# QData/ChromeGCN

Measured on AMD Instinct MI355X. Metric: GCN windows/sec (2-layer, d_model=128) on GM12878 Hi-C graph, higher is better.
Workload: dtype f32

## Files before the change

chromegcn_amd/_lib.py:

```python
import ctypes
import os

import torch

from . import _build

_c_int = ctypes.c_int
_c_vp = ctypes.c_void_p
_c_sz = ctypes.c_size_t
_c_float = ctypes.c_float
_c_uint = ctypes.c_uint

_TYPES = {"i": _c_int, "u": _c_uint, "ll": ctypes.c_longlong, "z": _c_sz, "f": _c_float, "zp": ctypes.POINTER(_c_sz)}
_HEADER = {
    "cgcn_abi_version": (_c_int, ""),
    "cgcn_strerror": (ctypes.c_char_p, "code:i"),
    "cgcn_spmm": (_c_int, "stream n_rows:i n_cols:i S:i d:i rowptr col val row_scale X Y aux"),
    "cgcn_layer_fwd": (_c_int, "stream n:i S:i d:i rowptr col val row_scale X W b wg cg Xn Z H gate dropout_p:f rng_state "
                               "stream_id:u H_in colstats colstats_rows:i aux"),
    "cgcn_layer_fwd_colstats_plan": (_c_int, "n:i S:i d:i mode:i rows_per_tile"),
    "cgcn_debug_set_fwd_split_bytes": (None, "bytes:ll"),
    "cgcn_debug_set_products": (None, "mode:i"),
    "cgcn_debug_get_products": (_c_int, ""),
    "cgcn_debug_layer_fwd_route": (_c_int, "n:i S:i d:i aux colstats_rows:i"),
    "cgcn_debug_layer_bwd_route": (_c_int, "n:i S:i d:i"),
    "cgcn_layer_bwd_workspace_bytes": (_c_sz, "n:i S:i d:i"),
    "cgcn_layer_bwd": (_c_int, "stream n:i S:i d:i rowptr_t col_t val_t row_scale X Z H gate W wg dXn dgate dX dHs dW db dwg "
                               "dcg accumulate:i in_dropout_p:f rng_state in_stream_id:u head workspace workspace_bytes:z "
                               "aux_stream sgd aux_t"),
    "cgcn_debug_layer_bwd_phases": (_c_int, "stream n:i S:i d:i rowptr_t col_t val_t row_scale X Z H gate W wg dXn dgate dX dHs "
                                            "dW db dwg dcg accumulate:i in_dropout_p:f rng_state in_stream_id:u head workspace "
                                            "workspace_bytes:z phases:i aux_t"),
    "cgcn_head_workspace_bytes": (_c_sz, "n:i S:i d:i C:i"),
    "cgcn_head_workspace_layout": (_c_int, "n:i S:i d:i C:i dym_offset:zp bnc_offset:zp part_offset:zp"),
    "cgcn_head_bwd_partials": (_c_int, "n:i"),
    "cgcn_head_fwd": (_c_int, "stream n:i S:i d:i C:i X bn_w bn_b run_mean run_var num_batches_tracked momentum:f eps:f "
                              "training:i W_out b_out target dropout_p:f rng_state probs loss dpred save_mean save_invstd "
                              "workspace workspace_bytes:z"),
    "cgcn_head_logits": (_c_int, "stream n:i S:i d:i C:i X bn_w bn_b run_mean run_var eps:f W_out b_out logits"),
    "cgcn_head_train": (_c_int, "stream n:i S:i d:i C:i X bn_w bn_b run_mean run_var num_batches_tracked momentum:f eps:f "
                                "W_out b_out target dropout_p:f rng_state probs loss save_mean save_invstd col_stats "
                                "col_stats_tiles:i col_stats_rows:i workspace workspace_bytes:z"),
    "cgcn_debug_head_train_phases": (_c_int, "stream n:i S:i d:i C:i X bn_w bn_b run_mean run_var num_batches_tracked "
                                             "momentum:f eps:f W_out b_out target dropout_p:f rng_state probs loss save_mean "
                                             "save_invstd col_stats col_stats_tiles:i col_stats_rows:i workspace "
                                             "workspace_bytes:z phases:i"),
    "cgcn_head_bwd": (_c_int, "stream n:i S:i d:i C:i X bn_w bn_b save_mean save_invstd W_out dpred dloss dropout_p:f "
                              "rng_state dX dW_out db_out dbn_w dbn_b accumulate:i workspace workspace_bytes:z"),
    "cgcn_sddmm": (_c_int, "stream n:i S:i d:i rowptr col A B out accumulate:i"),
    "cgcn_saliency_normalize": (_c_int, "stream n:i rowptr val raw out"),
    "cgcn_graph_count": (_c_int, "stream n:i adj_type:i rowptr_in col_in val_in row_counts rowptr_out"),
    "cgcn_graph_fill": (_c_int, "stream n:i adj_type:i rowptr_in col_in val_in rowptr_out col_out val_out row_scale "
                                "symmetric_flag"),
    "cgcn_metrics_workspace_bytes": (_c_sz, "n:ll C:i"),
    "cgcn_multilabel_metrics": (_c_int, "stream n:ll C:i probs targets fdr_cutoff:f out workspace workspace_bytes:z"),
    "cgcn_multilabel_metrics_nonneg": (_c_int, "stream n:ll C:i probs targets fdr_cutoff:f out bad workspace "
                                               "workspace_bytes:z"),
    "cgcn_sgd_step": (_c_int, "stream count:ll param grad momentum_buf lr:f momentum:f weight_decay:f nesterov:i "
                              "grad_scale:f rng_state"),
    "cgcn_adam_step": (_c_int, "stream count:ll param grad exp_avg exp_avg_sq step n_step:i ticket lr:f beta1:f beta2:f "
                               "eps:f weight_decay:f grad_scale:f rng_state"),
    "cgcn_ablation_prepare": (_c_int, "stream n:i C:i targets label_bits pos_lists pos_ranks pos_counts"),
    "cgcn_ablation_workspace_bytes": (_c_sz, "n_inst:i S:i d:i layers:i"),
    "cgcn_ablation_layer": (_c_int, "stream n:i S:i d:i rowptr col val row_scale X X_inst W b wg cg label_bits C:i pos_list "
                                    "pos_rank n_pos:i cols n_cols:i X_out removed"),
    "cgcn_ablation_head": (_c_int, "stream n:i S:i d:i C:i X X_inst bn_w bn_b run_mean run_var eps:f W_out b_out pos_lists "
                                   "pos_counts label:i n_pos:i cols n_cols:i removed base M"),
    "cgcn_ablation_mask": (_c_int, "stream n:i C:i rowptr col val row_scale label_bits label_i:i label_j:i val_out "
                                   "row_scale_out removed"),
    "cgcn_ablation_reduce": (_c_int, "stream n:i S:i C:i logits pos_lists pos_counts label:i col_label:i removed base M"),
    "cgcn_hic_workspace_bytes": (_c_sz, "M:ll N:i capacity:ll K:ll"),
    "cgcn_hic_count": (_c_int, "stream M:ll pos1 pos2 window_start N:i workspace workspace_bytes:z n_survivors"),
    "cgcn_hic_build": (_c_int, "stream M:ll pos1 pos2 count norm n_bins:ll resolution_bp:i window_start N:i K:ll capacity:ll "
                               "workspace workspace_bytes:z rowptr_out col_out nnz_out n_survivors"),
    "cgcn_hic_up_workspace_bytes": (_c_sz, "M:ll N:i capacity:ll K:ll resolution_bp:i window_bp:i n_window_bins:ll"),
    "cgcn_hic_count_up": (_c_int, "stream M:ll pos1 pos2 window_start N:i resolution_bp:i window_bp:i n_window_bins:ll workspace "
                                  "workspace_bytes:z n_survivors"),
    "cgcn_hic_build_up": (_c_int, "stream M:ll pos1 pos2 count norm n_bins:ll resolution_bp:i window_bp:i n_window_bins:ll "
                                  "window_start N:i K:ll capacity:ll workspace workspace_bytes:z rowptr_out col_out nnz_out "
                                  "n_survivors"),
    "cgcn_text_workspace_bytes": (_c_sz, "n_bytes:ll"),
    "cgcn_text_count": (_c_int, "stream text n_bytes:ll workspace workspace_bytes:z n_records"),
    "cgcn_text_parse": (_c_int, "stream text n_bytes:ll M:ll pos1_out pos2_out count_out flags flag_capacity:ll flag_totals "
                                "workspace workspace_bytes:z"),
}
_ABI = {fn: (res, tuple((p.partition(":")[0], _TYPES[p.partition(":")[2]] if ":" in p else _c_vp) for p in spec.split()))
        for fn, (res, spec) in _HEADER.items()}
_SIGNATURES = {fn: (res, [t for _, t in params]) for fn, (res, params) in _ABI.items()}
_PLANS = {fn: (tuple(p for p, _ in params), tuple(i for i, (_, t) in enumerate(params) if t in (_c_vp, _TYPES["zp"])),
               any(p == "stream" for p, _ in params))
          for fn, (_, params) in _ABI.items()}
ABI_VERSION = 26
COLSTATS_RECORDS, COLSTATS_ACCUMULATE = 0, 1
COLSTATS_ROWS_ACCUMULATE, COLSTATS_ROWS_ZERO_ONLY, COLSTATS_ROWS_ACCUMULATE_ZEROED = -1, -2, -3
_lib = None


class ChromeGCNLibraryError(RuntimeError):
    pass


def exported_symbols():
    return sorted(_SIGNATURES)


def load(build_if_missing=False):
    global _lib
    if _lib is not None:
        return _lib
    path = os.environ.get("CHROMEGCN_LIB") or _build.LIB
    if not os.path.exists(path):
        raise ChromeGCNLibraryError(
            "chromegcn_amd: %s is missing -- build it first: python -m chromegcn_amd._build (or "
            "__graft_entry__.build()).  There is no CPU/torch fallback for the HIP path." % path)
    if path == _build.LIB and _build.is_stale():
        raise ChromeGCNLibraryError(
            "chromegcn_amd: %s is stale (sources changed since it was built) -- rebuild: "
            "python -m chromegcn_amd._build" % path)
    _lib = open_library(path)
    return _lib


def open_library(path):
    lib = ctypes.CDLL(path)
    for name, (res, args) in _SIGNATURES.items():
        try:
            fn = getattr(lib, name)
        except AttributeError as e:
            raise ChromeGCNLibraryError("chromegcn_amd: symbol %s missing from %s" % (name, path)) from e
        fn.restype = res
        fn.argtypes = args
    got = lib.cgcn_abi_version()
    if got != ABI_VERSION:
        raise ChromeGCNLibraryError("chromegcn_amd: ABI version %d != expected %d; rebuild" % (got, ABI_VERSION))
    return lib


def check(rc, what):
    if rc != 0:
        msg = load().cgcn_strerror(rc).decode()
        raise RuntimeError("chromegcn_amd: %s failed: %s (code %d)" % (what, msg, rc))


def query(fn, **args):
    names, pointers, has_stream = _PLANS[fn]
    if has_stream and "stream" not in args:
        args["stream"] = stream_ptr()
    try:
        vals = list(map(args.__getitem__, names))
    except KeyError as e:
        raise TypeError("%s: missing argument %s" % (fn, e.args[0])) from None
    if len(args) != len(names):
        raise TypeError("%s: unknown argument(s) %s" % (fn, ", ".join(sorted(set(args) - set(names)))))
    for i in pointers:
        v = vals[i]
        if v.__class__ is torch.Tensor:
            vals[i] = v.data_ptr()
        elif v is not None and v.__class__ is not int:
            vals[i] = v.data_ptr() if isinstance(v, torch.Tensor) else ctypes.byref(v)
    return getattr(load(), fn)(*vals)


def call(fn, **args):
    check(query(fn, **args), fn)


def _workspace(nbytes, device, what):
    if nbytes == 0:
        raise RuntimeError("chromegcn_amd: %s: unsupported shape" % what)
    return torch.empty(nbytes, device=device, dtype=torch.uint8)


def head_workspace(n, S, d, C, device):
    return _workspace(query("cgcn_head_workspace_bytes", n=n, S=S, d=d, C=C), device,
                      "fused head, S=%d n=%d d=%d C=%d" % (S, n, d, C))


def layer_bwd_workspace(n, S, d, device):
    return _workspace(query("cgcn_layer_bwd_workspace_bytes", n=n, S=S, d=d), device,
                      "layer backward, S=%d n=%d d=%d" % (S, n, d))


class HeadGrad(ctypes.Structure):
    _fields_ = [("dym", _c_vp), ("bnc", _c_vp), ("save_mean", _c_vp), ("save_invstd", _c_vp), ("bn_w", _c_vp),
                ("dropout_p", _c_float), ("rng_state", _c_vp), ("part", _c_vp), ("n_partials", _c_int), ("C", _c_int),
                ("dW_out", _c_vp), ("db_out", _c_vp), ("accumulate", _c_int), ("dloss", _c_vp), ("dbn_w", _c_vp),
                ("dbn_b", _c_vp), ("stat_acc", _c_vp)]


class SgdFuse(ctypes.Structure):
    _fields_ = [("param", _c_vp), ("grad", _c_vp), ("momentum_buf", _c_vp), ("count", ctypes.c_longlong),
                ("lr", _c_float), ("momentum", _c_float), ("weight_decay", _c_float), ("grad_scale", _c_float),
                ("nesterov", _c_int), ("rng_state", _c_vp)]


def ptr(t):
    return None if t is None else t.data_ptr()


def stream_ptr():
    return torch.cuda.current_stream().cuda_stream


_aux_streams = {}


def aux_stream_ptr():
    if not os.environ.get("CHROMEGCN_AUX_STREAM"):
        return None
    dev = torch.cuda.current_device()
    s = _aux_streams.get(dev)
    if s is None:
        s = _aux_streams[dev] = torch.cuda.Stream(device=dev)
    return s.cuda_stream
```

chromegcn_amd/csrc/cgcn_kernels.hip:

```cpp
#include <atomic>
#include <type_traits>
#include <cstdlib>

#include "cgcn_common.hpp"

template <int S, int D>
struct Geo {
  static constexpr int PAY = S * D;
  static constexpr bool HALF = (PAY == 128);
  static constexpr int NV = HALF ? 1 : PAY / 256;
  static_assert(PAY == 128 || PAY == 256 || PAY == 512, "unsupported payload");
  __device__ static __forceinline__ int strand(int v, int lane) { return HALF ? 0 : ((v * 64 + lane) * 4) / D; }
  __device__ static __forceinline__ int column(int v, int lane) { return HALF ? (lane & 31) * 4 : ((v * 64 + lane) * 4) % D; }
};

#ifndef GU_OVERRIDE
#define GU_OVERRIDE 0
#endif
#ifndef NT_SAVED
#define NT_SAVED 0
#endif
#if NT_SAVED
#define NT_STORE4(p, v) __builtin_nontemporal_store((v), (f32x4*)(p))
#define NT_STORE1(p, v) __builtin_nontemporal_store((v), (p))
// ... 1791 lines not shown

template <int NT>
__device__ __forceinline__ void reduce_slab(int slab, int P, int D, const float* __restrict__ part,
                                            float* __restrict__ dW, float* __restrict__ db, float* __restrict__ dwg,
                                            float* __restrict__ dcg, int accumulate, const SgdFuse& sg) {
  constexpr int NS = NT / 64;
  const int PSTRIDE = D * D + 2 * D + 4;
  const int total = D * D + 2 * D + 1;
  __shared__ __attribute__((aligned(16))) float red[NS][64];
  const int lane = threadIdx.x & 63, wave = threadIdx.x >> 6;
  const int el4 = lane & 15, sub = lane >> 4;
  const int e0 = slab * 64 + el4 * 4;
  f32x4 a = {0.f, 0.f, 0.f, 0.f};
  if (e0 < total) {
    const int per = (P + NS * 4 - 1) / (NS * 4);
    const int p0 = (wave * 4 + sub) * per, p1 = min(P, p0 + per);
    for (int p = p0; p < p1; p += 8) {
      f32x4 t[8];
#pragma unroll
      for (int u = 0; u < 8; ++u) t[u] = *(const f32x4*)(part + (size_t)min(p + u, p1 - 1) * PSTRIDE + e0);
#pragma unroll
      for (int u = 0; u < 8; ++u)
        if (p + u < p1) a += t[u];
    }
  }
#pragma unroll
  for (int k = 0; k < 4; ++k) {
    float v = a[k];
    v += __shfl_xor(v, 16);
    v += __shfl_xor(v, 32);
    a[k] = v;
  }
  if (sub == 0) *(f32x4*)&red[wave][el4 * 4] = a;
  const int el = threadIdx.x & 63, slice = threadIdx.x >> 6;
  const int e = slab * 64 + el;
  float s;
  __syncthreads();
  if (slice == 0 && e < total) {
    s = 0.f;
#pragma unroll
    for (int w = 0; w < NS; ++w) s += red[w][el];
    float* dst;
    if (e < D * D) dst = dW + e;
    else if (e < D * D + D) dst = db + (e - D * D);
    else if (e < D * D + 2 * D) dst = dwg + (e - D * D - D);
    else dst = dcg;
    *dst = accumulate ? (*dst + s) : s;
    if (sg.param) sgd_apply(sg, (int)(dst - sg.grad), s);
  }
}

#ifndef REDUCE_WIDE_MAX_P
#define REDUCE_WIDE_MAX_P 64
#endif
template <int NT>
__device__ __forceinline__ void reduce_slab_wide(int wg, int P, int D, const float* __restrict__ part,
                                                 float* __restrict__ dW, float* __restrict__ db, float* __restrict__ dwg,
                                                 float* __restrict__ dcg, int accumulate, const SgdFuse& sg) {
  constexpr int NW = NT / 64;
  const int PSTRIDE = D * D + 2 * D + 4;
  const int total = D * D + 2 * D + 1;
  __shared__ __attribute__((aligned(16))) float redw[NW][256];
  const int lane = threadIdx.x & 63, wave = threadIdx.x >> 6;
  const int e0 = wg * 256 + lane * 4;
  f32x4 a = {0.f, 0.f, 0.f, 0.f};
  if (e0 < PSTRIDE) {
    const int per = (P + NW - 1) / NW;
    const int p0 = wave * per, p1 = min(P, p0 + per);
    for (int p = p0; p < p1; p += 8) {
      f32x4 t[8];
#pragma unroll
      for (int u = 0; u < 8; ++u) t[u] = *(const f32x4*)(part + (size_t)min(p + u, p1 - 1) * PSTRIDE + e0);
#pragma unroll
      for (int u = 0; u < 8; ++u)
        if (p + u < p1) a += t[u];
    }
  }
  *(f32x4*)&redw[wave][lane * 4] = a;
  __syncthreads();
  const int e = wg * 256 + (int)threadIdx.x;
  if (threadIdx.x < 256 && e < total) {
    float s = 0.f;
#pragma unroll
    for (int w = 0; w < NW; ++w) s += redw[w][threadIdx.x];
    float* dst;
    if (e < D * D) dst = dW + e;
    else if (e < D * D + D) dst = db + (e - D * D);
    else if (e < D * D + 2 * D) dst = dwg + (e - D * D - D);
    else dst = dcg;
    *dst = accumulate ? (*dst + s) : s;
    if (sg.param) sgd_apply(sg, (int)(dst - sg.grad), s);
  }
}

__device__ __forceinline__ void sgd_other_elements(const SgdFuse& sg, int block, int D, const float* dW, const float* db,
                                                   const float* dwg, const float* dcg) {
  const int i = block * (int)blockDim.x + (int)threadIdx.x;
  if (i == 0 && sg.rng_state) sg.rng_state[1] += 1ull;
  if (i < sg.count) {
    const float* gp = sg.grad + i;
    const bool mine = (gp >= dW && gp < dW + D * D) || (gp >= db && gp < db + D) || (gp >= dwg && gp < dwg + D) || gp == dcg;
    if (!mine) sgd_apply(sg, i, *gp);
  }
}

__global__ __launch_bounds__(256) void k_reduce_partials(int P, int D, const float* __restrict__ part,
                                                         float* __restrict__ dW, float* __restrict__ db,
                                                         float* __restrict__ dwg, float* __restrict__ dcg,
                                                         int accumulate, SgdFuse sg, int reduce_slabs) {
  if ((int)blockIdx.x >= reduce_slabs) {
    sgd_other_elements(sg, (int)blockIdx.x - reduce_slabs, D, dW, db, dwg, dcg);
    return;
  }
  reduce_slab<256>(blockIdx.x, P, D, part, dW, db, dwg, dcg, accumulate, sg);
}

#ifndef SLICED_HUB
#define SLICED_HUB 192
#endif
#ifndef SLICED_COST_MODEL
#define SLICED_COST_MODEL 1
#endif
#ifndef SLICED_COOP_OVERHEAD
#define SLICED_COOP_OVERHEAD 3
#endif
template <int U>
__device__ __forceinline__ int group8_bcast(int v) { return __builtin_amdgcn_ds_swizzle(v, 0x18 | (U << 5)); }

template <int U, bool HAS_VAL>
struct SlicedBcast {
  static __device__ __forceinline__ void run(unsigned (&off)[8], float (&w)[8], int myc, float myv, unsigned rowsh,
                                             unsigned lane_off) {
    SlicedBcast<U - 1, HAS_VAL>::run(off, w, myc, myv, rowsh, lane_off);
    off[U - 1] = ((unsigned)group8_bcast<U - 1>(myc) << rowsh) + lane_off;
    if (HAS_VAL) w[U - 1] = __int_as_float(group8_bcast<U - 1>(__float_as_int(myv)));
  }
};
template <bool HAS_VAL>
struct SlicedBcast<0, HAS_VAL> {
  static __device__ __forceinline__ void run(unsigned (&)[8], float (&)[8], int, float, unsigned, unsigned) {}
};

template <bool HAS_VAL, typename IT>
__device__ __forceinline__ f32x4 sliced_walk(const IT* __restrict__ col, const float* __restrict__ val, int k0, int k1,
                                             int step, const char* __restrict__ base, unsigned lane_off, unsigned rowsh, int j) {
  f32x4 acc = (f32x4){0.f, 0.f, 0.f, 0.f};
  for (int k = k0; k < k1; k += step) {
    const int kk = min(k + j, k1 - 1);
    const int myc = (int)col[kk];
    const float myv = HAS_VAL ? val[kk] : 0.f;
    unsigned off[8];
    float w[8];
    SlicedBcast<8, HAS_VAL>::run(off, w, myc, myv, rowsh, lane_off);
    f32x4 t[8];
#pragma unroll
    for (int u = 0; u < 8; ++u) t[u] = *(const f32x4*)(base + (size_t)off[u]);
    const f32x4 zero = (f32x4){0.f, 0.f, 0.f, 0.f};
#pragma unroll
    for (int u = 0; u < 8; ++u) {
      const f32x4 x = HAS_VAL ? w[u] * t[u] : t[u];
      acc += (k + u < k1) ? x : zero;
    }
  }
  return acc;
}

template <bool HAS_VAL, typename IT>
__device__ __forceinline__ f32x4 sliced_row_sum(const IT* __restrict__ col, const float* __restrict__ val, int k0, int k1,
                                                const char* __restrict__ base, unsigned lane_off, unsigned rowsh, int lane) {
  const int g = lane >> 3, j = lane & 7;
#if SLICED_COST_MODEL
  int mx = k1 - k0, sm = (k1 - k0 + 63) >> 6;
#pragma unroll
  for (int o = 8; o < 64; o <<= 1) {
    mx = max(mx, __shfl_xor(mx, o, WAVE));
    sm += __shfl_xor(sm, o, WAVE);
  }
  if (sm + SLICED_COOP_OVERHEAD >= ((mx + 7) >> 3)) return sliced_walk<HAS_VAL, IT>(col, val, k0, k1, 8, base, lane_off, rowsh, j);
#else
  if (!__any(k1 - k0 > SLICED_HUB)) return sliced_walk<HAS_VAL, IT>(col, val, k0, k1, 8, base, lane_off, rowsh, j);
#endif
  f32x4 mine = (f32x4){0.f, 0.f, 0.f, 0.f};
#pragma unroll 1
  for (int rr = 0; rr < 8; ++rr) {
    const int a0 = __shfl(k0, rr * 8, WAVE), a1 = __shfl(k1, rr * 8, WAVE);
    f32x4 acc = sliced_walk<HAS_VAL, IT>(col, val, a0 + g * 8, a1, 64, base, lane_off, rowsh, j);
#pragma unroll
    for (int e = 0; e < 4; ++e) {
      acc[e] += __shfl_xor(acc[e], 8, WAVE);
      acc[e] += __shfl_xor(acc[e], 16, WAVE);
      acc[e] += __shfl_xor(acc[e], 32, WAVE);
    }
    if (g == rr) mine = acc;
  }
  return mine;
}

#ifndef SLICED_SUPER
#define SLICED_SUPER 768
#endif
struct SlicedTile {
  int t0, t1;
  unsigned long long super;
  int i;
  int k0, k1;
  int g0;
};
__device__ __forceinline__ SlicedTile sliced_tile(const int* __restrict__ rowptr, const int* __restrict__ order, int n,
                                                  int tile, int wave, int lane) {
  SlicedTile t;
  const int r = tile * 64 + lane;
  int row = n;
  t.t0 = t.t1 = 0;
  if (r < n) {
    row = order ? order[r] : r;
    t.t0 = rowptr[row];
    t.t1 = rowptr[row + 1];
  }
  t.super = __ballot(t.t1 - t.t0 > SLICED_SUPER);
  t.g0 = __builtin_amdgcn_readfirstlane(row) & ~63;
  const int mine = wave * 8 + (lane >> 3);
  t.i = __shfl(row, mine, WAVE);
  t.k0 = __shfl(t.t0, mine, WAVE);
  t.k1 = __shfl(t.t1, mine, WAVE);
  return t;
}
template <bool HAS_VAL, typename IT>
__device__ __forceinline__ f32x4 sliced_super_sum(const IT* __restrict__ col, const float* __restrict__ val, const SlicedTile& t,
                                                  const char* __restrict__ base, unsigned lane_off, unsigned rowsh, int lane,
                                                  int wave) {
  __shared__ float s_part[8][32];
  __shared__ float s_res[64][32];
  const int g = lane >> 3, j = lane & 7;
  unsigned long long m = t.super;
  while (m) {
    const int r = __builtin_ctzll(m);
    m &= m - 1;
    const int a0 = __builtin_amdgcn_readlane(t.t0, r), a1 = __builtin_amdgcn_readlane(t.t1, r);
    const int seg = (((a1 - a0 + 7) >> 3) + 63) & ~63;
    const int w0 = a0 + wave * seg, w1 = min(a1, w0 + seg);
    f32x4 acc = sliced_walk<HAS_VAL, IT>(col, val, w0 + g * 8, w1, 64, base, lane_off, rowsh, j);
#pragma unroll
    for (int e = 0; e < 4; ++e) {
      acc[e] += __shfl_xor(acc[e], 8, WAVE);
      acc[e] += __shfl_xor(acc[e], 16, WAVE);
      acc[e] += __shfl_xor(acc[e], 32, WAVE);
    }
    if (lane < 8) *(f32x4*)&s_part[wave][lane * 4] = acc;
    __syncthreads();
    if (threadIdx.x < 32) {
      float x = s_part[0][threadIdx.x];
#pragma unroll
      for (int ww = 1; ww < 8; ++ww) x += s_part[ww][threadIdx.x];
      s_res[r][threadIdx.x] = x;
    }
    __syncthreads();
  }
  const bool super = (t.k1 - t.k0) > SLICED_SUPER;
  f32x4 mine = sliced_row_sum<HAS_VAL, IT>(col, val, t.k0, super ? t.k0 : t.k1, base, lane_off, rowsh, lane);
  if (super) mine = *(const f32x4*)&s_res[wave * 8 + g][j * 4];
  return mine;
}

#ifndef SLICED_NT
#define SLICED_NT 7
#endif
__device__ __forceinline__ f32x4 ld_stream4(const float* p) {
  if (SLICED_NT & 2) return __builtin_nontemporal_load((const f32x4*)p);
  return *(const f32x4*)p;
}
template <int NSL>
__device__ __forceinline__ void sliced_block(int b, int tiles, int& slice, int& tile) {
  if (NSL <= 8) {
    slice = b % NSL;
    tile = b / NSL;
  } else {
    const int per = 8 * tiles, pass = b / per, rem = b - pass * per;
    slice = (rem & 7) + 8 * pass;
    tile = rem >> 3;
  }
}

constexpr int BAND_W = 7;
constexpr int BANDPLUS_CHUNKS = (64 + 2 * BAND_W) * 8;
__device__ __forceinline__ void bandplus_stage(f32x4* __restrict__ bt, const float* __restrict__ T, size_t slice_el, int n, int g0, int D) {
  constexpr int NCH = BANDPLUS_CHUNKS;
#pragma unroll
  for (int u = 0; u < (NCH + 511) / 512; ++u) {
    const int idx = (int)threadIdx.x + 512 * u;
    const int j = g0 - BAND_W + (idx >> 3);
    f32x4 v = (f32x4){0.f, 0.f, 0.f, 0.f};
    if (idx < NCH && j >= 0 && j < n) v = *(const f32x4*)&T[slice_el + (size_t)j * D + (idx & 7) * 4];
    if (idx < NCH) bt[idx] = v;
  }
}
__device__ __forceinline__ f32x4 bandplus_sum(const f32x4* __restrict__ bt, int i, int g0, int lane) {
  const int li = i - g0, c = lane & 7;
  f32x4 a = (f32x4){0.f, 0.f, 0.f, 0.f};
#pragma unroll
  for (int k = 0; k <= 2 * BAND_W; ++k) a += bt[(li + k) * 8 + c];
  return a;
}

template <int S, int D, bool HAS_VAL, typename IT = int, bool BP = false>
__global__ __launch_bounds__(512) __attribute__((amdgpu_waves_per_eu(HAS_VAL ? 6 : 8))) void k_aggregate_sliced(int n, const int* __restrict__ rowptr, const IT* __restrict__ col,
                                                          const float* __restrict__ val, const float* __restrict__ rs,
                                                          const float* __restrict__ X, float* __restrict__ H,
                                                          const int* __restrict__ order,
                                                          unsigned long long* __restrict__ zero_words, int zero_count) {
  static_assert(!(BP && HAS_VAL), "the band-plus CSR holds unit entries");
  constexpr int NSL = S * D / 32, QPR = D / 32;
  const int lane = threadIdx.x & 63, wave = threadIdx.x >> 6;
  const int zblocks = (int)gridDim.x < 8 ? (int)gridDim.x : 8;
  if (zero_words && (int)blockIdx.x < zblocks)
    for (int i = (int)blockIdx.x * 512 + (int)threadIdx.x; i < zero_count; i += zblocks * 512) zero_words[i] = 0ull;
  int slice, tile;
  sliced_block<NSL>(blockIdx.x, (n + 63) / 64, slice, tile);
  const size_t slice_el = (size_t)(slice / QPR) * n * D + (slice % QPR) * 32;
  const size_t lane_el = slice_el + (lane & 7) * 4;
  const SlicedTile t = sliced_tile(rowptr, order, n, tile, wave, lane);
  __shared__ f32x4 bt[BP ? BANDPLUS_CHUNKS : 1];
  if (BP) {
    bandplus_stage(bt, X, slice_el, n, t.g0, D);
    __syncthreads();
  }
  const int i = t.i;
  const float sc = (i < n && rs) ? rs[i] : 1.f;
  const unsigned lane_off = (unsigned)(lane_el * 4), rowsh = D == 128 ? 9u : 10u;
  f32x4 acc = !t.super ? sliced_row_sum<HAS_VAL, IT>(col, val, t.k0, t.k1, (const char*)X, lane_off, rowsh, lane)
                       : sliced_super_sum<HAS_VAL, IT>(col, val, t, (const char*)X, lane_off, rowsh, lane, wave);
  if (i < n) {
    if (BP) acc += bandplus_sum(bt, i, t.g0, lane);
    if (SLICED_NT & 1) __builtin_nontemporal_store(acc * sc, (f32x4*)&H[lane_el + (size_t)i * D]);
    else *(f32x4*)&H[lane_el + (size_t)i * D] = acc * sc;
  }
}

template <int S, int D, bool EXT = false>
__device__ __forceinline__ void bwd_riders(int extra, int n, int P, const float* __restrict__ part, float* __restrict__ dW,
                                           float* __restrict__ db, float* __restrict__ dwg, float* __restrict__ dcg,
                                           int accumulate, const SgdFuse& sg, int reduce_slabs, const HeadApply& hp,
                                           int head_slabs, void* scratch = nullptr) {
  if (extra < reduce_slabs) {
    if (P <= REDUCE_WIDE_MAX_P) reduce_slab_wide<512>(extra, P, D, part, dW, db, dwg, dcg, accumulate, sg);
    else reduce_slab<512>(extra, P, D, part, dW, db, dwg, dcg, accumulate, sg);
    return;
  }
  extra -= reduce_slabs;
  if (extra < head_slabs) {
    const int wslabs = (hp.hf_CP * D + hp.hf_CP) / 64;
    if (extra < wslabs)
      head_finalize_slab<512, EXT>(extra, hp.hf_P, D, hp.hf_C, hp.hf_CP, hp.hf_part, hp.hf_dWout, hp.hf_dbout, hp.hf_accumulate, hp.dloss, scratch);
    else
      head_stats_finalize<512, EXT, 4>(extra - wslabs, hp.hf_P, n, S, D, hp.hf_CP, hp.hf_part, hp.hf_dbn_w, hp.hf_dbn_b, nullptr,
                                       hp.hf_accumulate, hp.dloss, scratch);
    return;
  }
  sgd_other_elements(sg, extra - head_slabs, D, dW, db, dwg, dcg);
}

template <int S, int D, bool HAS_VAL, typename IT = int, bool BP = false>
__global__ __launch_bounds__(512) __attribute__((amdgpu_waves_per_eu(HAS_VAL ? 6 : 8))) void k_bwd_sliced(int n, const int* __restrict__ rowptr, const IT* __restrict__ col,
                                                    const float* __restrict__ val, const float* __restrict__ dHs,
                                                    const float* dXn, const float* __restrict__ gate, float* dX,
                                                    float keep_scale, uint32_t thresh,
                                                    const unsigned long long* __restrict__ rng_state,
                                                    uint32_t stream_id, int gather_blocks, int P,
                                                    const float* __restrict__ part, float* __restrict__ dW,
                                                    float* __restrict__ db, float* __restrict__ dwg,
                                                    float* __restrict__ dcg, int accumulate, SgdFuse sg, int reduce_slabs,
                                                    const int* __restrict__ order, HeadApply hp, int head_slabs) {
  constexpr int RIDER_STAGE = 4 * (512 / HEAD_STAT_COLS) * (HEAD_STAT_COLS + 1) * (int)sizeof(double) / 16;
  __shared__ f32x4 bt[BP ? (BANDPLUS_CHUNKS > RIDER_STAGE ? BANDPLUS_CHUNKS : RIDER_STAGE) : 1];
  if ((int)blockIdx.x >= gather_blocks) {
#ifndef BSX_NORIDERS
    bwd_riders<S, D, BP>((int)blockIdx.x - gather_blocks, n, P, part, dW, db, dwg, dcg, accumulate, sg, reduce_slabs, hp, head_slabs, bt);
#endif
    return;
  }
  static_assert(!(BP && HAS_VAL), "the band-plus CSR holds unit entries");
  constexpr int NSL = S * D / 32, QPR = D / 32;
  const int lane = threadIdx.x & 63, wave = threadIdx.x >> 6;
  int slice, tile;
  sliced_block<NSL>(blockIdx.x, (n + 63) / 64, slice, tile);
  const int s = slice / QPR;
  const size_t slice_el = (size_t)s * n * D + (slice % QPR) * 32;
  const size_t lane_el = slice_el + (lane & 7) * 4;
  const SlicedTile t = sliced_tile(rowptr, order, n, tile, wave, lane);
  if (BP) {
    bandplus_stage(bt, dHs, slice_el, n, t.g0, D);
    __syncthreads();
  }
  const int i = t.i;
  const unsigned lane_off = (unsigned)(lane_el * 4), rowsh = D == 128 ? 9u : 10u;
  f32x4 res = (f32x4){0.f, 0.f, 0.f, 0.f}, acc;
  if (!t.super) {
#ifndef BSX_NODXN
    if (i < n) res = ld_stream4(&dXn[lane_el + (size_t)i * D]) * (1.f - gate[(size_t)s * n + i]);
#endif
    acc = sliced_row_sum<HAS_VAL, IT>(col, val, t.k0, t.k1, (const char*)dHs, lane_off, rowsh, lane);
  } else {
    acc = sliced_super_sum<HAS_VAL, IT>(col, val, t, (const char*)dHs, lane_off, rowsh, lane, wave);
    if (i < n) res = ld_stream4(&dXn[lane_el + (size_t)i * D]) * (1.f - gate[(size_t)s * n + i]);
  }
  if (BP && i < n) acc += bandplus_sum(bt, i, t.g0, lane);
  if (i >= n) return;
  const size_t g_off = lane_el + (size_t)i * D;
  f32x4 o = res + acc;
  if (thresh) {
    const uint32_t key = dropout_key(rng_state, stream_id);
#pragma unroll
    for (int e = 0; e < 4; ++e) o[e] = dropout_keep(key, (uint32_t)(g_off + e), thresh) ? o[e] * keep_scale : 0.f;
  }
#ifdef BSX_NOSTORE
  if (o[0] != 1.2345e33f) return;
#endif
  if (SLICED_NT & 4) __builtin_nontemporal_store(o, (f32x4*)&dX[g_off]);
  else *(f32x4*)&dX[g_off] = o;
}

#ifndef BAND_R
#define BAND_R 32
#endif
template <int D, int R>
struct BandGeo {
  static constexpr int CH = D / 4, RL = 512 / CH, RPT = R / RL, ROWS = R + 2 * BAND_W, NL = (ROWS * CH + 511) / 512;
  static constexpr int TROWS = NL * RL;
  static_assert(RL * RPT == R && RPT >= 1, "tile height is a multiple of the row lanes");
};
template <int D, int R>
__device__ __forceinline__ void band_tile_sums(const float* __restrict__ T, int n, int r0, float* __restrict__ tile,
                                               f32x4 (&acc)[BandGeo<D, R>::RPT]) {
  using G = BandGeo<D, R>;
  f32x4 v[G::NL];
  const int c0 = (int)threadIdx.x % G::CH, q0 = (int)threadIdx.x / G::CH;
#pragma unroll
  for (int u = 0; u < G::NL; ++u) {
    const int j = r0 - BAND_W + q0 + (512 / G::CH) * u;
    v[u] = *(const f32x4*)&T[(size_t)min(max(j, 0), n - 1) * D + 4 * c0];
  }
#pragma unroll
  for (int u = 0; u < G::NL; ++u) {
    const int row = q0 + (512 / G::CH) * u;
    const int j = r0 - BAND_W + row;
    const f32x4 z = (f32x4){0.f, 0.f, 0.f, 0.f};
    *(f32x4*)&tile[row * D + 4 * c0] = (j >= 0 && j < n) ? v[u] : z;
  }
  __syncthreads();
  const int c = (int)threadIdx.x % G::CH, rl = (int)threadIdx.x / G::CH;
#pragma unroll
  for (int p = 0; p < G::RPT; ++p) acc[p] = (f32x4){0.f, 0.f, 0.f, 0.f};
  const float* __restrict__ col = &tile[rl * G::RPT * D + 4 * c];
  constexpr int NK = G::RPT + 2 * BAND_W, KB = 4;
#pragma unroll
  for (int k0 = 0; k0 < NK; k0 += KB) {
    f32x4 w[KB];
#pragma unroll
    for (int u = 0; u < KB; ++u)
      if (k0 + u < NK) w[u] = *(const f32x4*)&col[(k0 + u) * D];
#pragma unroll
    for (int u = 0; u < KB; ++u)
#pragma unroll
      for (int p = 0; p < G::RPT; ++p)
        if (k0 + u < NK && k0 + u - p >= 0 && k0 + u - p <= 2 * BAND_W) acc[p] += w[u];
#pragma unroll
    for (int p = 0; p < G::RPT; ++p) asm volatile("" : "+v"(acc[p]));
  }
}

template <int S, int D, int R>
__global__ __launch_bounds__(512) __attribute__((amdgpu_waves_per_eu(8))) void k_band_aggregate(int n, const float* __restrict__ rs, const float* __restrict__ X,
                                                        float* __restrict__ H, unsigned long long* __restrict__ zero_words,
                                                        int zero_count) {
  using G = BandGeo<D, R>;
  const int zblocks = (int)gridDim.x < 8 ? (int)gridDim.x : 8;
  if (zero_words && (int)blockIdx.x < zblocks)
    for (int i = (int)blockIdx.x * 512 + (int)threadIdx.x; i < zero_count; i += zblocks * 512) zero_words[i] = 0ull;
  const int tiles = (n + R - 1) / R;
  const int b = xcd_contiguous((int)blockIdx.x, S * tiles);
  const int s = b / tiles, r0 = (b - s * tiles) * R;
  __shared__ __attribute__((aligned(16))) float tile[G::TROWS * D];
  f32x4 acc[G::RPT];
  band_tile_sums<D, R>(X + (size_t)s * n * D, n, r0, tile, acc);
  const int c = (int)threadIdx.x % G::CH, rl = (int)threadIdx.x / G::CH;
#pragma unroll
  for (int p = 0; p < G::RPT; ++p) {
    const int i = r0 + rl * G::RPT + p;
    if (i < n) {
      const f32x4 o = acc[p] * (rs ? rs[i] : 1.f);
      float* dst = &H[((size_t)s * n + i) * D + 4 * c];
      if (SLICED_NT & 1) __builtin_nontemporal_store(o, (f32x4*)dst);
      else *(f32x4*)dst = o;
    }
  }
}

template <int S, int D, int R>
__global__ __launch_bounds__(512) __attribute__((amdgpu_waves_per_eu(8))) void k_bwd_band(int n, const float* __restrict__ dHs, const float* dXn,
                                                  const float* __restrict__ gate, float* dX, float keep_scale, uint32_t thresh,
                                                  const unsigned long long* __restrict__ rng_state, uint32_t stream_id,
                                                  int gather_blocks, int P, const float* __restrict__ part,
                                                  float* __restrict__ dW, float* __restrict__ db, float* __restrict__ dwg,
                                                  float* __restrict__ dcg, int accumulate, SgdFuse sg, int reduce_slabs,
                                                  HeadApply hp, int head_slabs) {
  using G = BandGeo<D, R>;
  __shared__ __attribute__((aligned(16))) float tile[G::TROWS * D];
  static_assert(sizeof(tile) >= 4 * (512 / HEAD_STAT_COLS) * (HEAD_STAT_COLS + 1) * sizeof(double), "rider staging fits the tile");
  if ((int)blockIdx.x >= gather_blocks) {
    bwd_riders<S, D, true>((int)blockIdx.x - gather_blocks, n, P, part, dW, db, dwg, dcg, accumulate, sg, reduce_slabs, hp, head_slabs, tile);
    return;
  }
  const int tiles = (n + R - 1) / R;
  const int b = xcd_contiguous((int)blockIdx.x, gather_blocks);
  const int s = b / tiles, r0 = (b - s * tiles) * R;
  const int c = (int)threadIdx.x % G::CH, rl = (int)threadIdx.x / G::CH;
  f32x4 res[G::RPT];
#pragma unroll
  for (int p = 0; p < G::RPT; ++p) {
    const int i = r0 + rl * G::RPT + p;
    res[p] = (f32x4){0.f, 0.f, 0.f, 0.f};
    if (i < n) res[p] = ld_stream4(&dXn[((size_t)s * n + i) * D + 4 * c]) * (1.f - gate[(size_t)s * n + i]);
  }
  f32x4 acc[G::RPT];
  band_tile_sums<D, R>(dHs + (size_t)s * n * D, n, r0, tile, acc);
  const uint32_t key = thresh ? dropout_key(rng_state, stream_id) : 0u;
#pragma unroll
  for (int p = 0; p < G::RPT; ++p) {
    const int i = r0 + rl * G::RPT + p;
    if (i >= n) continue;
    const size_t g_off = ((size_t)s * n + i) * D + 4 * c;
    f32x4 o = res[p] + acc[p];
    if (thresh) {
#pragma unroll
      for (int e = 0; e < 4; ++e) o[e] = dropout_keep(key, (uint32_t)(g_off + e), thresh) ? o[e] * keep_scale : 0.f;
    }
    if (SLICED_NT & 4) __builtin_nontemporal_store(o, (f32x4*)&dX[g_off]);
    else *(f32x4*)&dX[g_off] = o;
  }
}

template <int S, int D>
__global__ __launch_bounds__(256) void k_sddmm(int n, const int* __restrict__ rowptr, const int* __restrict__ col,
                                               const float* __restrict__ A, const float* __restrict__ B,
                                               float* __restrict__ out, int accumulate) {
  using G = Geo<S, D>;
  constexpr int NV = G::NV;
  constexpr unsigned ROWB = D * 4;
  const int lane = threadIdx.x & 63;
  const int wave = blockIdx.x * (blockDim.x >> 6) + __builtin_amdgcn_readfirstlane(threadIdx.x >> 6);
  const int nwaves = (gridDim.x * blockDim.x) >> 6;
  unsigned lane_off[NV];
#pragma unroll
  for (int v = 0; v < NV; ++v) lane_off[v] = ((unsigned)G::strand(v, lane) * (unsigned)n * D + G::column(v, lane)) * 4u;
  for (int i = wave; i < n; i += nwaves) {
    f32x4 a[NV];
#pragma unroll
    for (int v = 0; v < NV; ++v) {
      a[v] = *(const f32x4*)((const char*)A + (size_t)i * ROWB + lane_off[v]);
      if (G::HALF && lane >= 32) a[v] = (f32x4){0.f, 0.f, 0.f, 0.f};
    }
    const int k0 = rowptr[i], k1 = rowptr[i + 1];
    for (int kb = k0; kb < k1; kb += WAVE) {
      const int cnt = min(WAVE, k1 - kb);
      const int myc = lane < cnt ? col[kb + lane] : 0;
      float mine = 0.f;
      for (int j = 0; j < cnt; j += 8) {
        f32x4 t[8][NV];
#pragma unroll
        for (int u = 0; u < 8; ++u) {
          const char* rowp = (const char*)B + (size_t)(unsigned)rl_i(myc, min(j + u, cnt - 1)) * ROWB;
#pragma unroll
          for (int v = 0; v < NV; ++v) {
            const unsigned off = G::HALF ? (unsigned)((lane & 31) * 16) : lane_off[v];
            t[u][v] = *(const f32x4*)(rowp + off);
          }
        }
#pragma unroll
        for (int u = 0; u < 8; ++u) {
          float d = 0.f;
#pragma unroll
          for (int v = 0; v < NV; ++v)
#pragma unroll
            for (int e = 0; e < 4; ++e) d += a[v][e] * t[u][v][e];
          d = wave_sum(d);
          if (lane == j + u) mine = d;
        }
      }
      if (lane < cnt) out[kb + lane] = accumulate ? out[kb + lane] + mine : mine;
    }
  }
}

__global__ __launch_bounds__(256) void k_saliency_rows(int n, const int* __restrict__ rowptr, const float* __restrict__ val,
                                                       const float* __restrict__ raw, float* __restrict__ out) {
  const int lane = threadIdx.x & 63;
  const int wave = blockIdx.x * (blockDim.x >> 6) + __builtin_amdgcn_readfirstlane(threadIdx.x >> 6);
  const int nwaves = (gridDim.x * blockDim.x) >> 6;
  for (int i = wave; i < n; i += nwaves) {
    const int k0 = rowptr[i], k1 = rowptr[i + 1];
    float s = 0.f;
    for (int kb = k0; kb < k1; kb += WAVE) {
      const int k = kb + lane;
      s += k < k1 ? fabsf((val ? val[k] : 1.f) * raw[k]) : 0.f;
    }
    s = wave_sum(s);
    if (s == 0.f) s = 1.f;
    float m = 0.f;
    for (int kb = k0; kb < k1; kb += WAVE) {
      const int k = kb + lane;
      m = fmaxf(m, k < k1 ? fabsf((val ? val[k] : 1.f) * raw[k]) / s : 0.f);
    }
#pragma unroll
    for (int o = 32; o > 0; o >>= 1) m = fmaxf(m, __shfl_xor(m, o, WAVE));
    if (m == 0.f) m = 1.f;
    for (int kb = k0; kb < k1; kb += WAVE) {
      const int k = kb + lane;
      if (k < k1) out[k] = fabsf((val ? val[k] : 1.f) * raw[k]) / s / m;
    }
  }
}

__global__ __launch_bounds__(256) void k_sgd(int count, float* __restrict__ p, const float* __restrict__ g,
                                             float* __restrict__ m, float lr, float mu, float wd, int nesterov,
                                             float grad_scale, unsigned long long* __restrict__ rng_state) {
  const int i = blockIdx.x * blockDim.x + threadIdx.x;
  if (i == 0 && rng_state) rng_state[1] += 1ull;
  if (i >= count) return;
  const float pi = p[i];
  float d = g[i] * grad_scale + wd * pi;
  float upd = d;
  if (m) {
    const float b = mu * m[i] + d;
    m[i] = b;
    upd = nesterov ? d + mu * b : b;
  }
  p[i] = pi - lr * upd;
}

__global__ __launch_bounds__(256) void k_adam(int count, float* __restrict__ p, const float* __restrict__ g,
                                              float* __restrict__ m, float* __restrict__ v, float* __restrict__ step,
                                              int n_step, int* __restrict__ ticket, float lr, float beta1, float beta2,
                                              float eps, float wd, float grad_scale, unsigned long long* __restrict__ rng_state) {
  __shared__ int last;
  const float t = step[0] + 1.f;
  const float bc1 = (float)(1.0 - pow((double)beta1, (double)t));
  const float bc2s = (float)sqrt(1.0 - pow((double)beta2, (double)t));
  const float step_size = lr / bc1;
  const float ob1 = 1.f - beta1, ob2 = 1.f - beta2;
  auto one = [&](float& pi, float gi, float& mi, float& vi) {
    const float d = gi * grad_scale + wd * pi;
    mi = mi + ob1 * (d - mi);
    vi = beta2 * vi + ob2 * d * d;
    const float denom = sqrtf(vi) / bc2s + eps;
    if (mi != 0.f) pi = pi - step_size * (mi / denom);
  };
  const int n4 = count >> 2;
  for (int i = blockIdx.x * blockDim.x + threadIdx.x; i < n4; i += gridDim.x * blockDim.x) {
    float4 pv = reinterpret_cast<float4*>(p)[i];
    const float4 gv = reinterpret_cast<const float4*>(g)[i];
    float4 mv = reinterpret_cast<float4*>(m)[i];
    float4 vv = reinterpret_cast<float4*>(v)[i];
    one(pv.x, gv.x, mv.x, vv.x);
    one(pv.y, gv.y, mv.y, vv.y);
    one(pv.z, gv.z, mv.z, vv.z);
    one(pv.w, gv.w, mv.w, vv.w);
    reinterpret_cast<float4*>(p)[i] = pv;
    reinterpret_cast<float4*>(m)[i] = mv;
    reinterpret_cast<float4*>(v)[i] = vv;
  }
  if (blockIdx.x == 0 && threadIdx.x < (count & 3)) {
    const int i = (n4 << 2) + threadIdx.x;
    one(p[i], g[i], m[i], v[i]);
  }
  if (blockIdx.x == 0 && threadIdx.x == 0 && rng_state) rng_state[1] += 1ull;
  asm volatile("s_waitcnt vmcnt(0) lgkmcnt(0)" ::: "memory");
  __syncthreads();
  if (threadIdx.x == 0)
    last = __hip_atomic_fetch_add(ticket, 1, __ATOMIC_RELAXED, __HIP_MEMORY_SCOPE_AGENT) == (int)gridDim.x - 1;
  __syncthreads();
  if (!last) return;
  for (int i = threadIdx.x; i < n_step; i += blockDim.x) step[i] = t;
  if (threadIdx.x == 0) __hip_atomic_store(ticket, 0, __ATOMIC_RELAXED, __HIP_MEMORY_SCOPE_AGENT);
}


static int check_shape(int n, int S, int d) {
  if (n < 0) return CGCN_ERR_BAD_ARG;
  if (!(S == 1 || S == 2) || !(d == 128 || d == 256)) return CGCN_ERR_UNSUPPORTED;
  if ((double)n * (double)S * (double)d * 4.0 >= 4294967296.0) return CGCN_ERR_UNSUPPORTED;
  return CGCN_OK;
}


#define DISPATCH_SDV(S_, d_, hasval_, CALL)                                      \
  do {                                                                           \
    if ((S_) == 1 && (d_) == 128) { if (hasval_) { CALL(1, 128, true); } else { CALL(1, 128, false); } } \
    else if ((S_) == 2 && (d_) == 128) { if (hasval_) { CALL(2, 128, true); } else { CALL(2, 128, false); } } \
    else if ((S_) == 1 && (d_) == 256) { if (hasval_) { CALL(1, 256, true); } else { CALL(1, 256, false); } } \
    else { if (hasval_) { CALL(2, 256, true); } else { CALL(2, 256, false); } }  \
  } while (0)

#ifndef DEEP_TABLE_BYTES
#define DEEP_TABLE_BYTES (12u << 20)
#endif
static inline bool pick_deep(int n, int S, int d) { return (double)n * S * d * 4.0 > (double)DEEP_TABLE_BYTES; }

static inline int pick_mb(int, int) { return 1; }

static hipEvent_t pooled_event() {
  struct Pool {
    hipEvent_t ev[64];
    Pool() {
      for (auto& e : ev)
        if (hipEventCreateWithFlags(&e, hipEventDisableTiming) != hipSuccess) e = nullptr;
    }
  };
  static Pool pool;
  static std::atomic<unsigned> next{0};
  return pool.ev[next.fetch_add(1u, std::memory_order_relaxed) & 63u];
}

static int dropout_args(float p, const unsigned long long* rng_state, float* keep_scale, uint32_t* thresh) {
  *keep_scale = 1.f;
  *thresh = 0u;
  if (p <= 0.f) return CGCN_OK;
  if (!rng_state || p >= 1.f) return CGCN_ERR_BAD_ARG;
  *keep_scale = 1.f / (1.f - p);
  *thresh = dropout_threshold(p);
  return CGCN_OK;
}

static void launch_aggregate_sliced(hipStream_t st, int gblocks, int n, int S, int d, const int32_t* rowptr, const int32_t* col,
                                    const uint16_t* col16, const float* val, const float* rs, const float* X, float* H,
                                    const int32_t* order, bool bp = false, unsigned long long* zero_words = nullptr,
                                    int zero_count = 0) {
#define SD4(CALLX)                         \
  do {                                     \
    if (S == 1 && d == 128) CALLX(1, 128); \
    else if (S == 2 && d == 128) CALLX(2, 128); \
    else if (S == 1 && d == 256) CALLX(1, 256); \
    else CALLX(2, 256);                    \
  } while (0)
  if (bp) {
#define CALLBP16(S_, D_) hipLaunchKernelGGL((k_aggregate_sliced<S_, D_, false, uint16_t, true>), dim3(gblocks), dim3(512), 0, st, n, rowptr, col16, nullptr, rs, X, H, order, zero_words, zero_count)
#define CALLBP32(S_, D_) hipLaunchKernelGGL((k_aggregate_sliced<S_, D_, false, int, true>), dim3(gblocks), dim3(512), 0, st, n, rowptr, col, nullptr, rs, X, H, order, zero_words, zero_count)
    if (col16) SD4(CALLBP16);
    else SD4(CALLBP32);
#undef CALLBP16
#undef CALLBP32
    return;
  }
  if (col16) {
#define CALL16(S_, D_) hipLaunchKernelGGL((k_aggregate_sliced<S_, D_, false, uint16_t>), dim3(gblocks), dim3(512), 0, st, n, rowptr, col16, val, rs, X, H, order, zero_words, zero_count)
    SD4(CALL16);
#undef CALL16
    return;
  }
#define CALL(S_, D_, V_) hipLaunchKernelGGL((k_aggregate_sliced<S_, D_, V_, int>), dim3(gblocks), dim3(512), 0, st, n, rowptr, col, val, rs, X, H, order, zero_words, zero_count)
  DISPATCH_SDV(S, d, val != nullptr, CALL);
#undef CALL
}
struct SlicedCsr {
  const int32_t* rowptr;
  const int32_t* col;
  const uint16_t* col16;
  const float* val;
  const int32_t* order;
  bool bp;
};
static inline SlicedCsr sliced_csr(const cgcn_graph_aux* aux, const int32_t* rowptr, const int32_t* col, const float* val, int n_cols);

extern "C" {

int cgcn_abi_version(void) { return CGCN_ABI_VERSION; }

const char* cgcn_strerror(int code) {
  switch (code) {
    case CGCN_OK: return "ok";
    case CGCN_ERR_BAD_ARG: return "bad argument (null pointer, negative size or misaligned buffer)";
    case CGCN_ERR_UNSUPPORTED: return "unsupported shape (need S in {1,2}; d in {128,256} for the fused kernels, a multiple of 4 <= 4096 for cgcn_spmm; S*n*d*4 < 4 GiB)";
    case CGCN_ERR_LAUNCH: return "HIP kernel launch failed";
    case CGCN_ERR_WORKSPACE: return "workspace too small";
    default: return "unknown chromegcn error";
  }
}

#ifndef FWD_SPLIT_TABLE_BYTES
#define FWD_SPLIT_TABLE_BYTES (6u << 20)
#endif
#ifndef DENSE_MAX_BLOCKS
#define DENSE_MAX_BLOCKS (256 * (DENSE_WAVES_PER_SIMD / 2))
#endif
static inline int dense_max_blocks(int d) { return d == 256 ? 256 : DENSE_MAX_BLOCKS; }
#ifndef DENSE_MB
#define DENSE_MB 1
#endif
static long long fwd_split_default() {
  const char* e = getenv("CGCN_FWD_SPLIT_BYTES");
  return (e && *e) ? atoll(e) : (long long)FWD_SPLIT_TABLE_BYTES;
}
static std::atomic<long long> g_fwd_split_bytes{fwd_split_default()};
void cgcn_debug_set_fwd_split_bytes(long long bytes) { g_fwd_split_bytes.store(bytes < 0 ? fwd_split_default() : bytes); }
static int products_default() {
  const char* e = getenv("CGCN_PRODUCTS");
  return (e && (e[0] == 'f' || e[0] == '0')) ? CGCN_PRODUCTS_FP32_CHAIN : CGCN_PRODUCTS_SPLIT;
}
static std::atomic<int> g_products{products_default()};
void cgcn_debug_set_products(int mode) {
  g_products.store((mode == CGCN_PRODUCTS_FP32_CHAIN || mode == CGCN_PRODUCTS_SPLIT) ? mode : products_default());
}
int cgcn_debug_get_products(void) { return g_products.load(); }

static inline const uint16_t* use_col16(const cgcn_graph_aux* aux, const float* val, int n_cols) {
  return (aux && aux->col16 && !val && n_cols <= 65536) ? aux->col16 : nullptr;
}
#ifndef FWD_HUB_ROW
#define FWD_HUB_ROW 2048
#endif
static inline bool hub_graph(const cgcn_graph_aux* aux) { return aux && aux->max_row_len > FWD_HUB_ROW; }
static inline const int32_t* row_order(const cgcn_graph_aux* aux) { return aux ? aux->row_order : nullptr; }
static inline SlicedCsr sliced_csr(const cgcn_graph_aux* aux, const int32_t* rowptr, const int32_t* col, const float* val, int n_cols) {
  if (aux && aux->bp_rowptr && aux->bp_col && val)
    return SlicedCsr{aux->bp_rowptr, aux->bp_col, n_cols <= 65536 ? aux->bp_col16 : nullptr, nullptr, aux->bp_row_order, true};
  return SlicedCsr{rowptr, col, use_col16(aux, val, n_cols), val, row_order(aux), false};
}
static inline bool band_graph(const cgcn_graph_aux* aux, const float* val) { return aux && aux->band_halfwidth == BAND_W && !val; }
static inline bool bandplus_graph(const cgcn_graph_aux* aux, const float* val) { return aux && aux->bp_rowptr && aux->bp_col && val; }
static void launch_band_aggregate(hipStream_t st, int n, int S, int d, const float* rs, const float* X, float* H,
                                  unsigned long long* zw = nullptr, int zc = 0) {
  const int blocks = S * ((n + BAND_R - 1) / BAND_R);
  if (S == 1 && d == 128) hipLaunchKernelGGL((k_band_aggregate<1, 128, BAND_R>), dim3(blocks), dim3(512), 0, st, n, rs, X, H, zw, zc);
  else if (S == 2 && d == 128) hipLaunchKernelGGL((k_band_aggregate<2, 128, BAND_R>), dim3(blocks), dim3(512), 0, st, n, rs, X, H, zw, zc);
  else if (S == 1 && d == 256) hipLaunchKernelGGL((k_band_aggregate<1, 256, BAND_R>), dim3(blocks), dim3(512), 0, st, n, rs, X, H, zw, zc);
  else hipLaunchKernelGGL((k_band_aggregate<2, 256, BAND_R>), dim3(blocks), dim3(512), 0, st, n, rs, X, H, zw, zc);
}

int cgcn_spmm(cgcn_stream_t stream, int n_rows, int n_cols, int S, int d, const int32_t* rowptr, const int32_t* col,
              const float* val, const float* row_scale, const float* X, float* Y, const cgcn_graph_aux* aux) {
  const int nmax = n_rows > n_cols ? n_rows : n_cols;
  if (nmax < 0) return CGCN_ERR_BAD_ARG;
  if (!(S == 1 || S == 2) || d < 4 || (d & 3) || d > 4096) return CGCN_ERR_UNSUPPORTED;
  if ((double)nmax * (double)S * (double)d * 4.0 >= 4294967296.0) return CGCN_ERR_UNSUPPORTED;
  if (n_rows == 0) return CGCN_OK;
  if (!rowptr || !col || !X || !Y || X == Y) return CGCN_ERR_BAD_ARG;
  if (misaligned16(X) || misaligned16(Y)) return CGCN_ERR_BAD_ARG;
  hipStream_t st = (hipStream_t)stream;
  if (!(d == 128 || d == 256)) {
    const long long rows = (long long)S * n_rows;
    const int blocks = (int)((rows + 3) / 4 < 8192 ? (rows + 3) / 4 : 8192);
    hipLaunchKernelGGL(k_spmm_any, dim3(blocks), dim3(256), 0, st, n_rows, n_cols, S, d, rowptr, col, val, row_scale, X, Y);
    return launch_status();
  }
  if (n_rows == n_cols && band_graph(aux, val)) {
    launch_band_aggregate(st, n_rows, S, d, row_scale, X, Y);
    return launch_status();
  }
  if (n_rows == n_cols && ((double)n_rows * S * d * 4.0 >= (double)g_fwd_split_bytes.load() || hub_graph(aux) || bandplus_graph(aux, val))) {
    const int gblocks = (S * d / 32) * ((n_rows + 63) / 64);
    const SlicedCsr c = sliced_csr(aux, rowptr, col, val, n_cols);
    launch_aggregate_sliced(st, gblocks, n_rows, S, d, c.rowptr, c.col, c.col16, c.val, row_scale, X, Y, c.order, c.bp);
    return launch_status();
  }
  const int blocks = (n_rows + 3) / 4 < 4096 ? (n_rows + 3) / 4 : 4096;
  const bool deep = false;
#define CALL(S_, D_, V_)                                                                                                  \
  do {                                                                                                                    \
    if (deep) hipLaunchKernelGGL((k_spmm<S_, D_, V_, true>), dim3(blocks), dim3(256), 0, st, n_rows, n_cols, rowptr, col, val, row_scale, X, Y); \
    else hipLaunchKernelGGL((k_spmm<S_, D_, V_, false>), dim3(blocks), dim3(256), 0, st, n_rows, n_cols, rowptr, col, val, row_scale, X, Y); \
  } while (0)
  DISPATCH_SDV(S, d, val != nullptr, CALL);
#undef CALL
  return launch_status();
}

static bool fwd_split_shape(int n, int S, int d) {
  const long long split_bytes = g_fwd_split_bytes.load();
  const double table = (double)n * S * d * 4.0;
  if (split_bytes == 0) return true;
  return table >= (double)split_bytes;
}
static int dense_stat_chunk(int n, int S, int d) {
  if (!fwd_split_shape(n, S, d)) return 1;
  const int tn = 16 * DENSE_MB / S;
  const int ntiles = (n + tn - 1) / tn;
  return (ntiles + dense_max_blocks(d) - 1) / dense_max_blocks(d);
}

static int acc_chunk(int n, int S, int d) {
  const int tn = 16 * DENSE_MB / S;
  const int ntiles = (n + tn - 1) / tn;
  return (ntiles + dense_max_blocks(d) - 1) / dense_max_blocks(d);
}

int cgcn_layer_fwd_colstats_plan(int n, int S, int d, int mode, int* rows_per_tile) {
  if (check_shape(n, S, d) != CGCN_OK || n == 0) return 0;
  if (mode != CGCN_COLSTATS_RECORDS && mode != CGCN_COLSTATS_ACCUMULATE) return 0;
  if (mode == CGCN_COLSTATS_ACCUMULATE && n >= 2) {
    if (rows_per_tile) *rows_per_tile = -1;
    const size_t tile_bytes = (size_t)S * d * 2 * sizeof(float);
    return (int)((stat_acc_words(S, d) * 8 + tile_bytes - 1) / tile_bytes);
  }
  const int tn = (16 * pick_mb(n, S) / S) * dense_stat_chunk(n, S, d);
  if (rows_per_tile) *rows_per_tile = tn;
  return (n + tn - 1) / tn;
}

int cgcn_debug_layer_fwd_route(int n, int S, int d, const cgcn_graph_aux* aux, int colstats_rows) {
  const int rc = check_shape(n, S, d);
  if (rc) return rc;
  if (band_graph(aux, nullptr)) return 2;
  const bool need_dense = colstats_rows == CGCN_COLSTATS_ROWS_ACCUMULATE || colstats_rows > 16 * DENSE_MB / S;
  return (fwd_split_shape(n, S, d) || hub_graph(aux) || (aux && aux->bp_rowptr && aux->bp_col) || need_dense) ? 1 : 0;
}

int cgcn_layer_fwd(cgcn_stream_t stream, int n, int S, int d, const int32_t* rowptr, const int32_t* col, const float* val,
                   const float* row_scale, const float* X, const float* W, const float* b, const float* wg,
                   const float* cg, float* Xn, float* Z, float* H, float* gate, float dropout_p,
                   const unsigned long long* rng_state, unsigned int stream_id, const float* H_in, float* colstats,
                   int colstats_rows, const cgcn_graph_aux* aux) {
  int rc = check_shape(n, S, d);
  if (rc) return rc;
  if (n == 0) return CGCN_OK;
  if (!rowptr || !col || !X || !W || !b || !wg || !cg || !Xn || !gate || X == Xn) return CGCN_ERR_BAD_ARG;
  if (misaligned16(X) || misaligned16(Xn) || misaligned16(W) || (Z && misaligned16(Z)) || (H && misaligned16(H)))
    return CGCN_ERR_BAD_ARG;
  if (H_in && (misaligned16(H_in) || H_in == H)) return CGCN_ERR_BAD_ARG;
  float ks;
  uint32_t th;
  if ((rc = dropout_args(dropout_p, rng_state, &ks, &th))) return rc;
  hipStream_t st = (hipStream_t)stream;
  const bool band = band_graph(aux, val);
  const int tn0 = 16 * DENSE_MB / S;
  const bool zero_only = colstats && colstats_rows == CGCN_COLSTATS_ROWS_ZERO_ONLY;
  const bool acc_pre = colstats && colstats_rows == CGCN_COLSTATS_ROWS_ACCUMULATE_ZEROED;
  const bool acc = colstats && (colstats_rows == CGCN_COLSTATS_ROWS_ACCUMULATE || acc_pre);
  int chunk = 1;
  if (colstats) {
    if (acc || zero_only) {
      if (n < 2 || ((uintptr_t)colstats & 7)) return CGCN_ERR_BAD_ARG;
      chunk = acc_chunk(n, S, d);
    } else {
      if (colstats_rows < tn0 || colstats_rows % tn0) return CGCN_ERR_BAD_ARG;
      chunk = colstats_rows / tn0;
    }
  }
  unsigned long long* zw = zero_only ? (unsigned long long*)colstats : nullptr;
  const int zc = zero_only ? (int)stat_acc_words(S, d) : 0;
  if (zero_only) colstats = nullptr;
  const bool need_dense = colstats && ((acc && !acc_pre) || (!acc && chunk != 1));
  const bool split = !H_in && H && (fwd_split_shape(n, S, d) || hub_graph(aux) || band || bandplus_graph(aux, val) || need_dense);
  if (!split && !H_in) chunk = 1;
  bool acc_zeroed = acc_pre;
  if (need_dense && !split && !H_in) return CGCN_ERR_BAD_ARG;
  if (split) {
    const int gblocks = (S * d / 32) * ((n + 63) / 64);
    unsigned long long* zq = zw ? zw : ((acc && !acc_pre) ? (unsigned long long*)colstats : nullptr);
    const int zn = zq ? (int)stat_acc_words(S, d) : 0;
    if (band) {
      launch_band_aggregate(st, n, S, d, row_scale, X, H, zq, zn);
    } else {
      const SlicedCsr c = sliced_csr(aux, rowptr, col, val, n);
      launch_aggregate_sliced(st, gblocks, n, S, d, c.rowptr, c.col, c.col16, c.val, row_scale, X, H, c.order, c.bp, zq, zn);
    }
    acc_zeroed = acc;
    zw = nullptr;
    if ((rc = launch_status())) return rc;
    H_in = H;
  }
  if (H_in) {
    if (acc && !acc_zeroed && hipMemsetAsync(colstats, 0, stat_acc_words(S, d) * 8, st) != hipSuccess) return CGCN_ERR_LAUNCH;
    constexpr int MB = DENSE_MB;
    const int tn = 16 * MB / S;
    const int ntiles = (n + tn - 1) / tn;
    const int grid = colstats ? (ntiles + chunk - 1) / chunk : (ntiles < dense_max_blocks(d) ? ntiles : dense_max_blocks(d));
    if (d == 256) {
      if (S == 1) hipLaunchKernelGGL((k_layer_dense256<1>), dim3(grid), dim3(1024), 0, st, n, ntiles, H_in, X, W, b, wg, cg, Xn, Z, gate,
                                     ks, th, rng_state, stream_id, colstats, chunk, acc ? 1 : 0, zw, zc);
      else hipLaunchKernelGGL((k_layer_dense256<2>), dim3(grid), dim3(1024), 0, st, n, ntiles, H_in, X, W, b, wg, cg, Xn, Z, gate,
                              ks, th, rng_state, stream_id, colstats, chunk, acc ? 1 : 0, zw, zc);
      return launch_status();
    }
    const bool sp = g_products.load() != CGCN_PRODUCTS_FP32_CHAIN;
#define CALL(S_, P_) \
    hipLaunchKernelGGL((k_layer_dense<S_, 128, MB, P_>), dim3(grid), dim3(512), 0, st, n, ntiles, H_in, X, W, b, wg, cg, Xn, Z, gate, \
                       ks, th, rng_state, stream_id, colstats, chunk, acc ? 1 : 0, zw, zc)
    if (S == 1) { if (sp) CALL(1, 1); else CALL(1, 0); }
    else { if (sp) CALL(2, 1); else CALL(2, 0); }
#undef CALL
    return launch_status();
  }
  const int mb = pick_mb(n, S);
  const int tn = 16 * mb / S;
  const int blocks = (n + tn - 1) / tn;
  const bool deep = pick_deep(n, S, d);
  const bool spf = g_products.load() != CGCN_PRODUCTS_FP32_CHAIN;
#define FWD(S_, D_, MB_, V_, DP_, P_)                                                                                 \
  hipLaunchKernelGGL((k_layer_fwd<S_, D_, MB_, V_, DP_, (D_ == 128) ? P_ : 0>), dim3(blocks), blk, 0, st, n, rowptr, col, val, row_scale, \
                     X, W, b, wg, cg, Xn, Z, H, gate, ks, th, rng_state, stream_id, colstats, acc ? 1 : 0, zw, zc)
#define CALL(S_, D_, V_)                                                                                              \
  do {                                                                                                                \
    const dim3 blk((D_ == 128 && CBW128 == 2) ? 256 : 512);                                                           \
    if (deep) { if (spf) FWD(S_, D_, 1, V_, true, 1); else FWD(S_, D_, 1, V_, true, 0); }                             \
    else { if (spf) FWD(S_, D_, 1, V_, false, 1); else FWD(S_, D_, 1, V_, false, 0); }                                \
  } while (0)
  DISPATCH_SDV(S, d, val != nullptr, CALL);
#undef CALL
#undef FWD
  return launch_status();
}

#ifndef BWD256_MAX_RANGES
#define BWD256_MAX_RANGES 64
#endif
static int bwd_partials(int n, int S, int d) {
  const int M = n * S;
  const int tr = d == 128 ? 16 : 32;
  const int ntiles = (M + tr - 1) / tr;
  if (d == 256) {
    const int nr = ((ntiles < BWD256_MAX_RANGES ? ntiles : BWD256_MAX_RANGES) + 7) / 8 * 8;
    return nr < 8 ? 8 : nr;
  }
  const int P = ntiles < BWD_MAX_PARTIALS ? ntiles : BWD_MAX_PARTIALS;
  return P < 1 ? 1 : P;
}

int cgcn_debug_layer_bwd_route(int n, int S, int d) {
  const int rc = check_shape(n, S, d);
  if (rc) return rc;
  return d == 128 ? 2 : 0;
}

size_t cgcn_layer_bwd_workspace_bytes(int n, int S, int d) {
  if (check_shape(n, S, d) != CGCN_OK) return 0;
  return (size_t)bwd_partials(n, S, d) * ((size_t)d * d + 2 * d + 4) * sizeof(float);
}

static int layer_bwd_impl(cgcn_stream_t stream, int n, int S, int d, const int32_t* rowptr_t, const int32_t* col_t,
                          const float* val_t, const float* row_scale, const float* X, const float* Z, const float* H,
                          const float* gate, const float* W, const float* wg, const float* dXn, const float* dgate, float* dX,
                          float* dHs, float* dW, float* db, float* dwg, float* dcg, int accumulate, float in_dropout_p,
                          const unsigned long long* rng_state, unsigned int in_stream_id, const cgcn_head_grad* head,
                          void* workspace, size_t workspace_bytes, cgcn_stream_t aux_stream, const cgcn_sgd_fuse* sgd,
                          int phases, const cgcn_graph_aux* aux_t) {
  int rc = check_shape(n, S, d);
  if (rc) return rc;
  if (!rowptr_t || !col_t || !X || !Z || !H || !gate || !W || !wg || !dW || !db || !dwg || !dcg) return CGCN_ERR_BAD_ARG;
  if (dX && !dHs) return CGCN_ERR_BAD_ARG;
  SgdFuse sg = {nullptr, nullptr, nullptr, 0, 0.f, 0.f, 0.f, 1.f, 0, nullptr};
  if (sgd) {
    if (n == 0 || accumulate || aux_stream) return CGCN_ERR_BAD_ARG;
    if (!sgd->param || !sgd->grad || sgd->count <= 0 || sgd->count > 2147483647LL) return CGCN_ERR_BAD_ARG;
    if ((sgd->momentum != 0.f) != (sgd->momentum_buf != nullptr) || (sgd->nesterov && sgd->momentum == 0.f)) return CGCN_ERR_BAD_ARG;
    const float* g0 = sgd->grad;
    const float* g1 = sgd->grad + sgd->count;
    if (!(dW >= g0 && dW + (size_t)d * d <= g1 && db >= g0 && db + d <= g1 && dwg >= g0 && dwg + d <= g1 && dcg >= g0 && dcg < g1))
      return CGCN_ERR_BAD_ARG;
    sg = SgdFuse{sgd->param, sgd->grad, sgd->momentum_buf, (int)sgd->count, sgd->lr, sgd->momentum, sgd->weight_decay,
                 sgd->grad_scale, sgd->nesterov, sgd->rng_state};
  }
  if ((dXn == nullptr) == (head == nullptr)) return CGCN_ERR_BAD_ARG;
  if (sgd && dX && in_dropout_p > 0.f) return CGCN_ERR_BAD_ARG;
  if ((dX && dX == dXn) || (dHs && (misaligned16(dHs) || dHs == dX)) || (dX && misaligned16(dX)) || misaligned16(W)) return CGCN_ERR_BAD_ARG;
  if (misaligned16(X) || misaligned16(Z) || misaligned16(H) || (dXn && misaligned16(dXn))) return CGCN_ERR_BAD_ARG;
  HeadApply hp = {nullptr, nullptr, nullptr, nullptr, nullptr, nullptr, nullptr, 1.f, 0u, S, nullptr, nullptr, nullptr, 0, 0, 0, 0, nullptr, nullptr, nullptr};
  int head_slabs = 0;
  if (head) {
    if (!head->dym || !head->bnc || !head->save_mean || !head->save_invstd || !head->bn_w) return CGCN_ERR_BAD_ARG;
    if (!head->part || !head->dW_out || !head->db_out || head->C < 1 || head->C > 256) return CGCN_ERR_BAD_ARG;
    float hks;
    uint32_t hth;
    if ((rc = dropout_args(head->dropout_p, head->rng_state, &hks, &hth))) return rc;
    const int CP = head->C <= 128 ? 128 : 256;
    if (head->stat_acc && ((uintptr_t)head->stat_acc & 7)) return CGCN_ERR_BAD_ARG;
    hp = HeadApply{head->dym, head->bnc, (const unsigned long long*)head->stat_acc, head->save_mean, head->save_invstd, head->bn_w, head->rng_state, hks, hth, S,
                   head->part, head->dW_out, head->db_out, head->n_partials, head->C, CP, head->accumulate, head->dloss,
                   head->dbn_w, head->dbn_b};
    if ((head->dbn_w == nullptr) != (head->dbn_b == nullptr)) return CGCN_ERR_BAD_ARG;
    head_slabs = (CP * d + CP) / 64 + (head->dbn_w ? d / HEAD_STAT_COLS : 0);
  }
#ifndef HEAD_SLABS_IN_GATHER
#define HEAD_SLABS_IN_GATHER 1
#endif
  const bool head_in_gather = HEAD_SLABS_IN_GATHER && head_slabs > 0 && n > 0 && dX != nullptr && !sg.param && !(aux_stream && aux_stream != stream);
  const int head_slabs_rl = head_in_gather ? 0 : head_slabs, head_slabs_g = head_in_gather ? head_slabs : 0;
  if (!workspace || workspace_bytes < cgcn_layer_bwd_workspace_bytes(n, S, d)) return CGCN_ERR_WORKSPACE;
  if (misaligned16(workspace)) return CGCN_ERR_BAD_ARG;
  float ks;
  uint32_t th;
  if ((rc = dropout_args(in_dropout_p, rng_state, &ks, &th))) return rc;
  hipStream_t st = (hipStream_t)stream;
  const int P = bwd_partials(n, S, d);
  float* part = (float*)workspace;
  const int M = n * S;
  if (!(phases & 1)) {
  } else if (d == 128) {
    const bool spb = g_products.load() != CGCN_PRODUCTS_FP32_CHAIN;
#define RING_(H_, D_, P_) hipLaunchKernelGGL((k_bwd_rowlocal_ring<H_, D_, P_>), dim3(P + head_slabs_rl), dim3(RING_THREADS), 0, st, M, n, dXn, Z, X, gate, dgate, H, wg, row_scale, dHs, part, hp, dX, P, head_slabs_rl, W)
#define RING(H_, D_) do { if (spb) RING_(H_, D_, 1); else RING_(H_, D_, 0); } while (0)
    if (!head) RING(false, false);
    else if (hp.thresh) RING(true, true);
    else RING(true, false);
#undef RING
#undef RING_
  } else
    hipLaunchKernelGGL((k_bwd_rowlocal256s<32>), dim3(4 * P + head_slabs_rl), dim3(RL256_THREADS), 0, st, M, n, dXn, Z, X, gate, dgate, H, wg, row_scale, dHs, part, hp, dX, 4 * P, head_slabs_rl, W);
  if ((rc = launch_status())) return rc;
  if (!(phases & 2)) return CGCN_OK;
  const int total = d * d + 2 * d + 1;
  hipStream_t rs_stream = st;
  hipEvent_t ev_fork = nullptr, ev_join = nullptr;
  if (aux_stream && aux_stream != stream && n > 0) {
    ev_fork = pooled_event();
    ev_join = pooled_event();
    if (ev_fork && ev_join && hipEventRecord(ev_fork, st) == hipSuccess &&
        hipStreamWaitEvent((hipStream_t)aux_stream, ev_fork, 0) == hipSuccess)
      rs_stream = (hipStream_t)aux_stream;
  }
  const int slabs = (total + 63) / 64;
  const int rslabs = P <= REDUCE_WIDE_MAX_P ? (total + 255) / 256 : slabs;
  const bool fuse_reduce = (rs_stream == st) && n > 0 && dX != nullptr;
  if (!fuse_reduce) {
    const int sgd_blocks_r = sg.param ? (sg.count + 255) / 256 : 0;
    hipLaunchKernelGGL(k_reduce_partials, dim3(slabs + sgd_blocks_r), dim3(256), 0, rs_stream, P, d, part, dW, db, dwg, dcg,
                       accumulate, sg, slabs);
    if ((rc = launch_status())) return rc;
    if (rs_stream != st && hipEventRecord(ev_join, rs_stream) != hipSuccess) return CGCN_ERR_LAUNCH;
  }
  if (n == 0 || !dX) {
    if (rs_stream != st && hipStreamWaitEvent(st, ev_join, 0) != hipSuccess) return CGCN_ERR_LAUNCH;
    return CGCN_OK;
  }
  const int blocks = (S * d / 32) * ((n + 63) / 64);
  if (head) dXn = dX;
  const int sgd_blocks = sg.param ? (sg.count + 511) / 512 : 0;
  if (band_graph(aux_t, val_t)) {
    const int bblocks = S * ((n + BAND_R - 1) / BAND_R);
#define CALLB(S_, D_)                                                                                                 \
  hipLaunchKernelGGL((k_bwd_band<S_, D_, BAND_R>), dim3(bblocks + (fuse_reduce ? rslabs : 0) + head_slabs_g + sgd_blocks), dim3(512), 0, st, \
                     n, dHs, dXn, gate, dX, ks, th, rng_state, in_stream_id, bblocks, P, part, dW, db, dwg, dcg, accumulate, sg, \
                     fuse_reduce ? rslabs : 0, hp, head_slabs_g)
    if (S == 1 && d == 128) CALLB(1, 128);
    else if (S == 2 && d == 128) CALLB(2, 128);
    else if (S == 1 && d == 256) CALLB(1, 256);
    else CALLB(2, 256);
#undef CALLB
  } else if (bandplus_graph(aux_t, val_t)) {
    const SlicedCsr c = sliced_csr(aux_t, rowptr_t, col_t, val_t, n);
#define CALLBP(S_, D_, IT_, COL_)                                                                                    \
  hipLaunchKernelGGL((k_bwd_sliced<S_, D_, false, IT_, true>), dim3(blocks + (fuse_reduce ? rslabs : 0) + head_slabs_g + sgd_blocks), dim3(512), 0, \
                     st, n, c.rowptr, COL_, nullptr, dHs, dXn, gate, dX, ks, th, rng_state, in_stream_id, blocks, P,  \
                     part, dW, db, dwg, dcg, accumulate, sg, fuse_reduce ? rslabs : 0, c.order, hp, head_slabs_g)
#define CALLBP16(S_, D_) CALLBP(S_, D_, uint16_t, c.col16)
#define CALLBP32(S_, D_) CALLBP(S_, D_, int, c.col)
    if (c.col16) { if (S == 1 && d == 128) CALLBP16(1, 128); else if (S == 2 && d == 128) CALLBP16(2, 128); else if (S == 1 && d == 256) CALLBP16(1, 256); else CALLBP16(2, 256); }
    else { if (S == 1 && d == 128) CALLBP32(1, 128); else if (S == 2 && d == 128) CALLBP32(2, 128); else if (S == 1 && d == 256) CALLBP32(1, 256); else CALLBP32(2, 256); }
#undef CALLBP16
#undef CALLBP32
#undef CALLBP
  } else if (const uint16_t* col16_t = use_col16(aux_t, val_t, n)) {
#define CALL16(S_, D_)                                                                                               \
  hipLaunchKernelGGL((k_bwd_sliced<S_, D_, false, uint16_t>), dim3(blocks + (fuse_reduce ? rslabs : 0) + head_slabs_g + sgd_blocks), dim3(512), 0, \
                     st, n, rowptr_t, col16_t, val_t, dHs, dXn, gate, dX, ks, th, rng_state, in_stream_id, blocks, P, \
                     part, dW, db, dwg, dcg, accumulate, sg, fuse_reduce ? rslabs : 0, row_order(aux_t), hp, head_slabs_g)
    if (S == 1 && d == 128) CALL16(1, 128);
    else if (S == 2 && d == 128) CALL16(2, 128);
    else if (S == 1 && d == 256) CALL16(1, 256);
    else CALL16(2, 256);
#undef CALL16
  } else {
#define CALL(S_, D_, V_)                                                                                             \
  hipLaunchKernelGGL((k_bwd_sliced<S_, D_, V_, int>), dim3(blocks + (fuse_reduce ? rslabs : 0) + head_slabs_g + sgd_blocks), dim3(512), 0, \
                     st, n, rowptr_t, col_t, val_t, dHs, dXn, gate, dX, ks, th, rng_state, in_stream_id, blocks, P,  \
                     part, dW, db, dwg, dcg, accumulate, sg, fuse_reduce ? rslabs : 0, row_order(aux_t), hp, head_slabs_g)
    DISPATCH_SDV(S, d, val_t != nullptr, CALL);
#undef CALL
  }
  if ((rc = launch_status())) return rc;
  if (rs_stream != st && hipStreamWaitEvent(st, ev_join, 0) != hipSuccess) return CGCN_ERR_LAUNCH;
  return CGCN_OK;
}

int cgcn_layer_bwd(cgcn_stream_t stream, int n, int S, int d, const int32_t* rowptr_t, const int32_t* col_t,
                   const float* val_t, const float* row_scale, const float* X, const float* Z, const float* H,
                   const float* gate, const float* W, const float* wg, const float* dXn, const float* dgate, float* dX,
                   float* dHs, float* dW, float* db, float* dwg, float* dcg, int accumulate, float in_dropout_p,
                   const unsigned long long* rng_state, unsigned int in_stream_id, const cgcn_head_grad* head,
                   void* workspace, size_t workspace_bytes, cgcn_stream_t aux_stream, const cgcn_sgd_fuse* sgd,
                   const cgcn_graph_aux* aux_t) {
  return layer_bwd_impl(stream, n, S, d, rowptr_t, col_t, val_t, row_scale, X, Z, H, gate, W, wg, dXn, dgate, dX, dHs, dW, db,
                        dwg, dcg, accumulate, in_dropout_p, rng_state, in_stream_id, head, workspace, workspace_bytes,
                        aux_stream, sgd, 3, aux_t);
}

int cgcn_debug_layer_bwd_phases(cgcn_stream_t stream, int n, int S, int d, const int32_t* rowptr_t, const int32_t* col_t,
                                const float* val_t, const float* row_scale, const float* X, const float* Z, const float* H,
                                const float* gate, const float* W, const float* wg, const float* dXn, const float* dgate,
                                float* dX, float* dHs, float* dW, float* db, float* dwg, float* dcg, int accumulate,
                                float in_dropout_p, const unsigned long long* rng_state, unsigned int in_stream_id,
                                const cgcn_head_grad* head, void* workspace, size_t workspace_bytes, int phases,
                                const cgcn_graph_aux* aux_t) {
  if (phases < 1 || phases > 3) return CGCN_ERR_BAD_ARG;
  return layer_bwd_impl(stream, n, S, d, rowptr_t, col_t, val_t, row_scale, X, Z, H, gate, W, wg, dXn, dgate, dX, dHs, dW, db,
                        dwg, dcg, accumulate, in_dropout_p, rng_state, in_stream_id, head, workspace, workspace_bytes,
                        nullptr, nullptr, phases, aux_t);
}

int cgcn_sddmm(cgcn_stream_t stream, int n, int S, int d, const int32_t* rowptr, const int32_t* col, const float* A,
               const float* B, float* out, int accumulate) {
  int rc = check_shape(n, S, d);
  if (rc) return rc;
  if (n == 0) return CGCN_OK;
  if (!rowptr || !col || !A || !B || !out || misaligned16(A) || misaligned16(B)) return CGCN_ERR_BAD_ARG;
  hipStream_t st = (hipStream_t)stream;
  const int blocks = (n + 3) / 4 < 4096 ? (n + 3) / 4 : 4096;
  if (S == 1 && d == 128) hipLaunchKernelGGL((k_sddmm<1, 128>), dim3(blocks), dim3(256), 0, st, n, rowptr, col, A, B, out, accumulate);
  else if (S == 2 && d == 128) hipLaunchKernelGGL((k_sddmm<2, 128>), dim3(blocks), dim3(256), 0, st, n, rowptr, col, A, B, out, accumulate);
  else if (S == 1 && d == 256) hipLaunchKernelGGL((k_sddmm<1, 256>), dim3(blocks), dim3(256), 0, st, n, rowptr, col, A, B, out, accumulate);
  else hipLaunchKernelGGL((k_sddmm<2, 256>), dim3(blocks), dim3(256), 0, st, n, rowptr, col, A, B, out, accumulate);
  return launch_status();
}

int cgcn_saliency_normalize(cgcn_stream_t stream, int n, const int32_t* rowptr, const float* val, const float* raw, float* out) {
  if (n < 0) return CGCN_ERR_BAD_ARG;
  if (n == 0) return CGCN_OK;
  if (!rowptr || !raw || !out) return CGCN_ERR_BAD_ARG;
  const int blocks = (n + 3) / 4 < 4096 ? (n + 3) / 4 : 4096;
  hipLaunchKernelGGL(k_saliency_rows, dim3(blocks), dim3(256), 0, (hipStream_t)stream, n, rowptr, val, raw, out);
  return launch_status();
}

int cgcn_sgd_step(cgcn_stream_t stream, long long count, float* param, const float* grad, float* momentum_buf, float lr,
                  float momentum, float weight_decay, int nesterov, float grad_scale, unsigned long long* rng_state) {
  if (count < 0 || count > 2147483647LL) return CGCN_ERR_UNSUPPORTED;
  if (count > 0 && (!param || !grad)) return CGCN_ERR_BAD_ARG;
  if (momentum != 0.f && !momentum_buf) return CGCN_ERR_BAD_ARG;
  if (nesterov && momentum == 0.f) return CGCN_ERR_BAD_ARG;
  hipStream_t st = (hipStream_t)stream;
  const int blocks = count > 0 ? (int)((count + 255) / 256) : 1;
  hipLaunchKernelGGL(k_sgd, dim3(blocks), dim3(256), 0, st, (int)count, param, grad, momentum != 0.f ? momentum_buf : nullptr,
                     lr, momentum, weight_decay, nesterov, grad_scale, rng_state);
  return launch_status();
}

int cgcn_adam_step(cgcn_stream_t stream, long long count, float* param, const float* grad, float* exp_avg, float* exp_avg_sq,
                   float* step, int n_step, int32_t* ticket, float lr, float beta1, float beta2, float eps,
                   float weight_decay, float grad_scale, unsigned long long* rng_state) {
  if (count < 0 || n_step < 1) return CGCN_ERR_BAD_ARG;
  if (count > 2147483647LL) return CGCN_ERR_UNSUPPORTED;
  if (!step || !ticket) return CGCN_ERR_BAD_ARG;
  if (count > 0 && (!param || !grad || !exp_avg || !exp_avg_sq)) return CGCN_ERR_BAD_ARG;
  if (misaligned16(param) || misaligned16(grad) || misaligned16(exp_avg) || misaligned16(exp_avg_sq)) return CGCN_ERR_BAD_ARG;
  if (!(beta1 >= 0.f && beta1 < 1.f) || !(beta2 >= 0.f && beta2 < 1.f) || !(eps >= 0.f)) return CGCN_ERR_BAD_ARG;
  const long long n4 = count / 4;
  long long blocks = (n4 + 255) / 256;
  if (blocks < 1) blocks = 1;
  if (blocks > 1024) blocks = 1024;
  hipLaunchKernelGGL(k_adam, dim3((unsigned)blocks), dim3(256), 0, (hipStream_t)stream, (int)count, param, grad, exp_avg,
                     exp_avg_sq, step, n_step, (int*)ticket, lr, beta1, beta2, eps, weight_decay, grad_scale, rng_state);
  return launch_status();
}

}
```

chromegcn_amd/finetune.py:

```python
from __future__ import annotations

import gc
import os
import pickle
import time
import weakref
from typing import Dict, Iterable, List, Optional, Sequence

import torch
import torch.nn.functional as F

from . import _lib as _lib_mod
from . import graph as G
from .dist import ShardPlan, plan_shards


class _Chrom:
    __slots__ = ("name", "n", "graph", "x", "target", "cost", "h1", "src_key", "stat_acc")

    def __init__(self, name, n, graph, x, target, cost, src_key=None, stat_acc=False):
        self.name, self.n, self.graph, self.x, self.target, self.cost = name, n, graph, x, target, cost
        self.stat_acc = bool(stat_acc)
        self.h1 = {"h": None}
        self.src_key = src_key


class _SourceKey:
    __slots__ = ("refs", "versions", "hic_ref", "hic_sig")

    def __init__(self, feats, hic):
        self.refs, self.versions = [], []
        for k in ("forward", "backward", "target"):
            t = feats[k]
            try:
                self.refs.append(weakref.ref(t))
            except TypeError:
                self.refs.append(None)
            self.versions.append(t._version if torch.is_tensor(t) else None)
        self.hic_ref = None
        if hic is not None:
            try:
                self.hic_ref = weakref.ref(hic)
            except TypeError:
                self.hic_ref = lambda: None
        self.hic_sig = None if hic is None else (getattr(hic, "nnz", None), getattr(hic, "shape", None))

    def matches(self, feats, hic) -> bool:
        for r, v, k in zip(self.refs, self.versions, ("forward", "backward", "target")):
            t = feats[k]
            if r is None or r() is not t or (torch.is_tensor(t) and t._version != v):
                return False
        if hic is None:
            return self.hic_ref is None
        if self.hic_ref is None or self.hic_ref() is not hic:
            return False
        return self.hic_sig == (getattr(hic, "nnz", None), getattr(hic, "shape", None))


def _graph_uses(key, name) -> bool:
    return key[0] == name or (isinstance(key[0], tuple) and name in key[0])


class _HostArena:

    def __init__(self, rows: int, C: int, device):
        self.device = device
        self.bufs = []
        for _ in range(2):
            try:
                self.bufs.append(torch.empty((rows, C), dtype=torch.float32, pin_memory=True))
            except RuntimeError:
                self.bufs.append(torch.empty((rows, C), dtype=torch.float32))
        self.turn = 0
        self.stream = torch.cuda.Stream(device=device)
        self.events: List[torch.cuda.Event] = []
        self.used = 0

    def begin(self):
        self.turn ^= 1
        self.used = 0

    def fetch(self, rows_list, probs_dev):
        if self.used == len(self.events):
            self.events.append(torch.cuda.Event())
        ev = self.events[self.used]
        self.used += 1
        ev.record(torch.cuda.current_stream(self.device))
        self.stream.wait_event(ev)
        runs = []
        for r0, r1 in rows_list:
            if runs and runs[-1][1] == r0:
                runs[-1][1] = r1
            else:
                runs.append([r0, r1])
        with torch.cuda.stream(self.stream):
            for r0, r1 in runs:
                self.bufs[self.turn][r0:r1].copy_(probs_dev[r0:r1], non_blocking=True)

    def finish(self, span, rows_list):
        self.stream.synchronize()
        buf = self.bufs[self.turn]
        if span is not None:
            return buf[span[0]:span[1]]
        return torch.cat([buf[r0:r1] for r0, r1 in rows_list], 0)


class GCNStage:

    def __init__(self, model, optimizer=None, adj_type: str = "hic", device="cuda", hip_graphs: bool = True,
                 input_grad: bool = False, group=None, fused_head: bool = True, cache_input_aggregation: bool = True,
                 force_collectives: bool = False, group_graph: Optional[bool] = None, p2p_allreduce: Optional[bool] = None,
                 prediction_gather: str = "all", aux_group=None, epoch_graph: Optional[bool] = None,
                 stat_acc: Optional[bool] = None):
        self.model = model
        self.stat_acc = stat_acc if stat_acc is not None else (None if os.environ.get("CGCN_STAT_ACC", "1") != "0" else False)
        self.epoch_graph = epoch_graph if epoch_graph is not None else os.environ.get("CGCN_EPOCH_GRAPH", "1") != "0"
        if prediction_gather not in ("all", "rank0", "none"):
            raise ValueError("prediction_gather must be 'all', 'rank0' or 'none'")
        self.prediction_gather = prediction_gather
        self.prediction_gather_effective = prediction_gather
        self._group_graph_opt = group_graph if group_graph is not None else os.environ.get("CGCN_GROUP_GRAPH", "1") != "0"
        self._group_graph_ok = True
        self._comm_warm = False
        self._p2p_opt = p2p_allreduce if p2p_allreduce is not None else os.environ.get("CGCN_P2P_ALLREDUCE", "0") == "1"
        self._p2p = None
        self.allreduce_kind = "none"
        self.fused_head = fused_head
        self.cache_input_aggregation = cache_input_aggregation
        self.optimizer = optimizer
        self.adj_type = adj_type
        self.device = torch.device(device)
        self.hip_graphs = bool(hip_graphs) and self.device.type == "cuda"
        self.input_grad = input_grad
        self.group = group
        if group is not None or (torch.distributed.is_available() and torch.distributed.is_initialized()):
            self.world = torch.distributed.get_world_size(group)
            self.rank = torch.distributed.get_rank(group)
        else:
            self.world, self.rank = 1, 0
        if force_collectives and not (torch.distributed.is_available() and torch.distributed.is_initialized()):
            raise RuntimeError("force_collectives needs an initialised torch.distributed process group")
        self.multi = self.world > 1 or bool(force_collectives)
        self.aux_group = aux_group if aux_group is not None else group
        if (self.multi and aux_group is None and group in (None, getattr(torch.distributed.group, "WORLD", None))
                and torch.distributed.is_available() and torch.distributed.is_initialized()
                and os.environ.get("CGCN_AUX_GROUP", "1") != "0"):
            self.aux_group = torch.distributed.new_group(backend=torch.distributed.get_backend(group))
        self.chroms: Dict[str, _Chrom] = {}
        self._pending: Dict[str, tuple] = {}
        self._meta: Dict[str, tuple] = {}
        self._graphs: Dict[tuple, dict] = {}
        self._pool = None
        self._flat_grad: Optional[torch.Tensor] = None
        self._flat_param: Optional[torch.Tensor] = None
        self._flat_mom: Optional[torch.Tensor] = None
        self._flat_m: Optional[torch.Tensor] = None
        self._flat_v: Optional[torch.Tensor] = None
        self._flat_step: Optional[torch.Tensor] = None
        self._ticket: Optional[torch.Tensor] = None
        self._fused: Optional[str] = None
        self._captured_lr = None
        self._one: Optional[torch.Tensor] = None
        self._targets_cpu: Dict[tuple, torch.Tensor] = {}
        self._gather_plans: Dict[tuple, dict] = {}
        self._targets_dev: Dict[tuple, torch.Tensor] = {}
        self._arena: Optional[dict] = None

    def _drop_graphs(self):
        self._graphs.clear()
        self._pool = None

    def add_chromosome(self, name: str, feats: Dict[str, torch.Tensor], hic=None, defer: bool = False):
        n = feats["forward"].shape[0]
        cost = self._cost_estimate(hic, n, feats["forward"].shape[1])
        if defer:
            self._pending[name] = (feats, hic)
            self._meta[name] = (n, feats["target"].shape[1], cost)
            self.chroms.pop(name, None)
            self._invalidate_layout(name)
            return
        pend = self._pending.pop(name, None)
        materialising = pend is not None and pend[0] is feats and pend[1] is hic
        if isinstance(hic, G.ChromGraph):
            if hic.n != n or hic.device.type != self.device.type:
                raise ValueError("graph of %s has %d windows on %s; the features have %d rows on %s"
                                 % (name, hic.n, hic.device, n, self.device))
            g = hic
        else:
            g = G.upload(G.normalize_graph(self.adj_type, hic, n), self.device)
        x = torch.stack([feats["forward"], feats["backward"]]).to(self.device, torch.float32).contiguous()
        t = feats["target"].to(self.device, torch.float32).contiguous()
        known = self._meta.get(name)
        self.chroms[name] = _Chrom(name, n, g, x, t, cost, _SourceKey(feats, hic), self._stat_acc_for(name, n, x))
        if known is None or known[:2] != (n, t.shape[1]):
            self._meta[name] = (n, t.shape[1], cost)
            self._invalidate_layout(name)
        else:
            if known[2] != cost:
                self._gather_plans.clear()
            self._meta[name] = (n, t.shape[1], cost)
            self._graphs = {k: v for k, v in self._graphs.items() if not _graph_uses(k, name)}
            if not materialising:
                self._targets_cpu.clear()
                self._targets_dev.clear()

    def _stat_acc_for(self, name: str, n: int, x: torch.Tensor) -> bool:
        if self.stat_acc is not None:
            return bool(self.stat_acc)
        if n < 2 or x.numel() == 0 or x.device.type != "cuda":
            return False
        keep = 1.0 / max(1e-6, 1.0 - float(getattr(self.model, "dropout", 0.0) or 0.0))
        bound = max(1.0, float(x.abs().max())) * keep ** max(int(getattr(self.model, "n_layers", 1)) - 1, 0)
        ok = n * bound * bound < 2.0 ** 29
        if not ok:
            import warnings
            warnings.warn("chromegcn_amd: feature magnitudes up to %.3g on the %d windows of %s are outside the range of the "
                          "fixed-point BatchNorm sums; this chromosome uses per-workgroup records" % (bound, n, name))
        return ok

    def _cost_estimate(self, hic, n: int, d: int) -> float:
        nnz = n
        if self.adj_type in ("hic", "both") and hic is not None and hasattr(hic, "nnz"):
            nnz += int(hic.nnz)
        if self.adj_type in ("constant", "both"):
            nnz += 14 * n
        return float(nnz) * d + 3.0 * n * d * d / 16.0

    def _invalidate_layout(self, name):
        self._targets_cpu.clear()
        self._targets_dev.clear()
        self._gather_plans.clear()
        self._arena = None
        self._graphs = {k: v for k, v in self._graphs.items() if not _graph_uses(k, name)}
        if not self._graphs:
            self._pool = None

    def _resident(self, name: str) -> _Chrom:
        c = self.chroms.get(name)
        if c is None:
            feats, hic = self._pending[name]
            self.add_chromosome(name, feats, hic)
            c = self.chroms[name]
        return c

    def load(self, chrom_feature_dict, split_adj_dict=None, only: Optional[Iterable[str]] = None, defer: bool = False):
        for name in chrom_feature_dict:
            if only is not None and name not in only:
                continue
            hic = None if split_adj_dict is None else split_adj_dict.get(name)
            cur = self.chroms.get(name)
            if cur is not None and cur.src_key is not None and cur.src_key.matches(chrom_feature_dict[name], hic):
                continue
            pend = self._pending.get(name)
            if defer and pend is not None and pend[0] is chrom_feature_dict[name] and pend[1] is hic:
                continue
            self.add_chromosome(name, chrom_feature_dict[name], hic, defer=defer)

    def invalidate(self, name: Optional[str] = None):
        for nm in ([name] if name is not None else list(self._meta)):
            self.chroms.pop(nm, None)
            self._pending.pop(nm, None)
            self._meta.pop(nm, None)
            self._graphs = {k: v for k, v in self._graphs.items() if not _graph_uses(k, nm)}
        if not self._graphs:
            self._pool = None
        self._targets_cpu.clear()
        self._targets_dev.clear()
        self._gather_plans.clear()
        self._arena = None

    def _ensure_arena(self):
        if self._arena is not None or not self._meta:
            return
        C = next(iter(self._meta.values()))[1]
        total = sum(m[0] for m in self._meta.values())
        probs = torch.empty((total, C), device=self.device, dtype=torch.float32)
        loss = torch.zeros(len(self._meta), device=self.device, dtype=torch.float32)
        slots, rows, order = {}, {}, {}
        off = 0
        for i, (nm, (n_, _c, _cost)) in enumerate(self._meta.items()):
            slots[nm] = {"probs": probs[off:off + n_], "loss": loss[i:i + 1]}
            rows[nm] = (off, off + n_)
            order[nm] = i
            off += n_
        self._arena = {"probs": probs, "loss": loss, "slots": slots, "rows": rows, "order": order}
        self._drop_graphs()

    def _arena_span(self, names):
        if not names:
            return None
        order = self._arena["order"]
        idx = [order[nm] for nm in names]
        if idx != list(range(idx[0], idx[0] + len(idx))):
            return None
        return self._arena["rows"][names[0]][0], self._arena["rows"][names[-1]][1], idx[0], idx[-1] + 1

    def _params(self):
        return [p for p in self.model.parameters() if p.requires_grad]

    def _fused_kind(self, ps):
        o = self.optimizer
        if o is None or type(o) not in (torch.optim.SGD, torch.optim.Adam) or len(o.param_groups) != 1 or self.device.type != "cuda":
            return None
        g = o.param_groups[0]
        if not (len(g["params"]) == len(ps) and all(a is b for a, b in zip(g["params"], ps))):
            return None
        if type(o) is torch.optim.SGD:
            return "sgd" if g.get("dampening", 0) == 0 and not g.get("maximize", False) else None
        return "adam" if self._adam_eligible(g, ps) else None

    def _adam_eligible(self, g, ps) -> bool:
        if not (g.get("fused") or g.get("capturable")):
            return False
        if g.get("amsgrad") or g.get("maximize") or g.get("differentiable") or g.get("decoupled_weight_decay", False):
            return False
        if any(torch.is_tensor(x) for x in (g["lr"], g["eps"], g["weight_decay"], *g["betas"])):
            return False
        if self._adam_adopted(ps):
            return True
        sts = [self.optimizer.state.get(p) for p in ps]
        if not any(sts):
            return True
        for p, st in zip(ps, sts):
            if not st or set(st) != {"step", "exp_avg", "exp_avg_sq"}:
                return False
            if not all(torch.is_tensor(st[k]) and st[k].shape == p.shape for k in ("exp_avg", "exp_avg_sq")):
                return False
        steps = torch.stack([torch.as_tensor(st["step"]).detach().to("cpu", torch.float64).reshape(()) for st in sts])
        return bool((steps == steps[0]).all())

    def _adam_adopted(self, ps) -> bool:
        if self._flat_step is None or self._flat_step.numel() != len(ps):
            return False
        offs, total = self._offsets(ps)
        if self._flat_m.numel() != total:
            return False
        bs, bm, bv = self._flat_step.data_ptr(), self._flat_m.data_ptr(), self._flat_v.data_ptr()
        for i, (p, off) in enumerate(zip(ps, offs)):
            st = self.optimizer.state.get(p)
            if not st:
                return False
            s, m, v = st.get("step"), st.get("exp_avg"), st.get("exp_avg_sq")
            if not (torch.is_tensor(s) and torch.is_tensor(m) and torch.is_tensor(v)):
                return False
            if s.data_ptr() != bs + 4 * i or m.data_ptr() != bm + 4 * off or v.data_ptr() != bv + 4 * off:
                return False
        return True

    def _adopt_adam_state(self, ps, offs, total, dev):
        self._flat_m = torch.zeros(total, device=dev, dtype=torch.float32)
        self._flat_v = torch.zeros(total, device=dev, dtype=torch.float32)
        self._flat_step = torch.zeros(len(ps), device=dev, dtype=torch.float32)
        if self._ticket is None or self._ticket.device != dev:
            self._ticket = torch.zeros(1, device=dev, dtype=torch.int32)
        for i, (p, off) in enumerate(zip(ps, offs)):
            st = self.optimizer.state[p]
            m = self._flat_m[off:off + p.numel()].view(p.shape)
            v = self._flat_v[off:off + p.numel()].view(p.shape)
            if "step" in st:
                self._flat_step[i].copy_(torch.as_tensor(st["step"]).reshape(()))
            if torch.is_tensor(st.get("exp_avg")):
                m.copy_(st["exp_avg"])
            if torch.is_tensor(st.get("exp_avg_sq")):
                v.copy_(st["exp_avg_sq"])
            st["step"], st["exp_avg"], st["exp_avg_sq"] = self._flat_step[i], m, v

    @staticmethod
    def _offsets(ps):
        offs, off = [], 0
        for p in ps:
            offs.append(off)
            off += (p.numel() + 3) & ~3
        return offs, off

    def _views_ok(self, ps, flat, attr):
        offs, total = self._offsets(ps)
        if flat is None or flat.numel() != total or flat.device != ps[0].device:
            return False
        for p, off in zip(ps, offs):
            t = p.data if attr == "data" else p.grad
            if t is None or t.data_ptr() != flat.data_ptr() + 4 * off or not t.is_contiguous():
                return False
        return True

    def _ensure_flat_grad(self):
        ps = self._params()
        offs, total = self._offsets(ps)
        dev = ps[0].device
        ok = self._views_ok(ps, self._flat_param, "data") and self._views_ok(ps, self._flat_grad, "grad")
        kind = self._fused_kind(ps)
        if ok and self._fused == kind and (kind != "adam" or self._adam_adopted(ps)):
            return
        with torch.no_grad():
            flat_p = torch.zeros(total, device=dev, dtype=torch.float32)
            for p, off in zip(ps, offs):
                flat_p[off:off + p.numel()].copy_(p.data.reshape(-1))
                p.data = flat_p[off:off + p.numel()].view(p.shape)
            self._flat_param = flat_p
            self._flat_grad = self._alloc_flat_grad(total, dev)
            for p, off in zip(ps, offs):
                p.grad = self._flat_grad[off:off + p.numel()].view(p.shape)
            self._fused = kind
            self._flat_mom = None
            self._flat_m = self._flat_v = self._flat_step = None
            if kind == "adam":
                self._adopt_adam_state(ps, offs, total, dev)
            if kind == "sgd" and self.optimizer.param_groups[0].get("momentum", 0) != 0:
                self._flat_mom = torch.zeros(total, device=dev, dtype=torch.float32)
                for p, off in zip(ps, offs):
                    st = self.optimizer.state[p]
                    view = self._flat_mom[off:off + p.numel()].view(p.shape)
                    if torch.is_tensor(st.get("momentum_buffer")):
                        view.copy_(st["momentum_buffer"])
                    st["momentum_buffer"] = view
        managed = dev.type == "cuda" and hasattr(self.model, "_rng_state")
        self.model._rng_managed = managed
        self.model._grad_sink = dev.type == "cuda" and hasattr(self.model, "forward_loss") and self.fused_head
        self._drop_graphs()

    def _optimizer_step(self, grad_scale: float = 1.0):
        rng = self.model._rng_state if getattr(self.model, "_rng_managed", False) else None
        if self._fused == "sgd":
            from . import ops
            g = self.optimizer.param_groups[0]
            ops.sgd_step(self._flat_param, self._flat_grad, self._flat_mom, g["lr"], g.get("momentum", 0),
                         g.get("weight_decay", 0), g.get("nesterov", False), rng, grad_scale)
        elif self._fused == "adam":
            from . import ops
            g = self.optimizer.param_groups[0]
            ops.adam_step(self._flat_param, self._flat_grad, self._flat_m, self._flat_v, self._flat_step, self._ticket,
                          g["lr"], g["betas"][0], g["betas"][1], g["eps"], g["weight_decay"], rng, grad_scale)
        else:
            if grad_scale != 1.0:
                self._flat_grad.mul_(grad_scale)
            self.optimizer.step()
            if rng is not None:
                rng[1] += 1

    def _forward_loss(self, c: _Chrom, x):
        slot = self._arena["slots"][c.name] if self._arena is not None else None
        if self.fused_head and hasattr(self.model, "forward_loss"):
            loss, probs, _ = self.model.forward_loss(x, c.graph, c.target,
                                                     h1_cache=c.h1 if self.cache_input_aggregation else None,
                                                     out_slots=slot, stat_acc=c.stat_acc)
            return loss, probs
        logits, _ = self.model.forward_strands(x, c.graph)
        pred = (logits[0] + logits[1]) / 2
        loss = F.binary_cross_entropy_with_logits(pred, c.target)
        if slot is None:
            return loss, torch.sigmoid(pred).detach()
        with torch.no_grad():
            torch.sigmoid(pred, out=slot["probs"])
            slot["loss"].copy_(loss.detach().view(1))
        return loss, slot["probs"]

    def _fwd_bwd_step(self, c: _Chrom):
        from . import ops
        fuse = self._fused == "sgd" and getattr(self.model, "_grad_sink", False) and getattr(self.model, "n_layers", 0) >= 1
        if fuse:
            g = self.optimizer.param_groups[0]
            ops._sgd_fuse = {"param": self._flat_param, "grad": self._flat_grad, "mom": self._flat_mom, "lr": g["lr"],
                             "momentum": g.get("momentum", 0), "weight_decay": g.get("weight_decay", 0),
                             "nesterov": g.get("nesterov", False), "grad_scale": 1.0, "done": False,
                             "rng_state": self.model._rng_state if getattr(self.model, "_rng_managed", False) else None}
        try:
            out = self._fwd_bwd(c)
            done = bool(fuse and ops._sgd_fuse["done"])
        finally:
            ops._sgd_fuse = None
        if not done:
            self._optimizer_step()
        return out

    def _fwd_bwd(self, c: _Chrom):
        x = c.x.detach().requires_grad_(True) if self.input_grad else c.x
        if not getattr(self.model, "_grad_sink", False):
            self._flat_grad.zero_()
        loss, probs = self._forward_loss(c, x)
        if self._one is None or self._one.device != loss.device:
            self._one = torch.ones((), device=loss.device)
        loss.backward(self._one)
        return loss.detach(), probs, (x.grad if self.input_grad else None)

    def _eval(self, c: _Chrom):
        with torch.no_grad():
            loss, probs = self._forward_loss(c, c.x)
        return loss, probs

    def _snapshot(self):
        st = {"model": {k: v.clone() for k, v in self.model.state_dict().items()}}
        rng = getattr(self.model, "_rng_state", None)
        if torch.is_tensor(rng):
            st["rng"] = rng.clone()
        if self.optimizer is not None:
            st["opt"] = [{k: (v.clone() if torch.is_tensor(v) else v) for k, v in s.items()}
                         for s in (self.optimizer.state.get(p, {}) for p in self._params())]
        return st

    def _restore(self, st):
        with torch.no_grad():
            for k, v in self.model.state_dict().items():
                v.copy_(st["model"][k])
            if "rng" in st:
                self.model._rng_state.copy_(st["rng"])
            if self.optimizer is not None:
                for p, saved in zip(self._params(), st["opt"]):
                    cur = self.optimizer.state.get(p, {})
                    for k, v in cur.items():
                        if torch.is_tensor(v):
                            if k in saved and torch.is_tensor(saved[k]):
                                v.copy_(saved[k])
                            else:
                                v.zero_()

    def _lr_signature(self):
        if self.optimizer is None:
            return None
        return tuple((g.get("lr"), g.get("momentum"), g.get("weight_decay"), g.get("nesterov"),
                      tuple(g["betas"]) if "betas" in g else None, g.get("eps")) for g in self.optimizer.param_groups)

    def _capture(self, c: Optional[_Chrom], kind: str, group_size: int = 1):
        was_training = self.model.training
        self.model.train(kind not in ("eval", "epoch_eval"))
        snap = self._snapshot()

        def body(collective=True):
            if kind in ("epoch", "epoch_eval"):
                out = None
                for cc in c:
                    out = self._fwd_bwd_step(cc) if kind == "epoch" else self._eval(cc) + (None,)
                return out
            if kind == "eval":
                loss, probs = self._eval(c)
                return loss, probs, None
            if kind == "train":
                return self._fwd_bwd_step(c)
            if kind == "group":
                if c is not None:
                    out = self._fwd_bwd(c)
                else:
                    self._flat_grad.zero_()
                    out = (None, None, None)
                if collective:
                    self._allreduce_grads()
                self._optimizer_step(1.0 / group_size if group_size > 1 else 1.0)
                return out
            return self._fwd_bwd(c)

        if kind in ("train", "epoch") and not self._fused:
            raise RuntimeError("only the fused SGD / Adam step can be captured; use kind='fwdbwd' + an eager optimizer.step()")
        try:
            side = torch.cuda.Stream(device=self.device)
            side.wait_stream(torch.cuda.current_stream(self.device))
            with torch.cuda.stream(side):
                for _ in range(2):
                    body(collective=False)
            torch.cuda.current_stream(self.device).wait_stream(side)
            torch.cuda.synchronize(self.device)
            self._restore(snap)
            graph = torch.cuda.CUDAGraph()
            if self._pool is None:
                self._pool = torch.cuda.graph_pool_handle()
            gc_was_enabled = gc.isenabled()
            gc.disable()
            try:
                with torch.cuda.graph(graph, pool=self._pool, capture_error_mode="thread_local"):
                    loss, probs, dx = body()
            finally:
                if gc_was_enabled:
                    gc.enable()
        finally:
            self._restore(snap)
            self.model.train(was_training)
        return {"graph": graph, "loss": loss, "probs": probs, "dx": dx}

    def _replay(self, c: Optional[_Chrom], kind: str, group_size: int = 1):
        if self._captured_lr != self._lr_signature():
            self._drop_graphs()
            self._captured_lr = self._lr_signature()
        key = (c.name if c is not None else None, kind) if kind != "group" else (c.name if c is not None else None, kind, group_size)
        ent = self._graphs.get(key)
        if ent is None:
            ent = self._graphs[key] = self._capture(c, kind, group_size)
        ent["graph"].replay()
        return ent["loss"], ent["probs"], ent["dx"]

    def _replay_epoch(self, names, train: bool) -> bool:
        if not (self.epoch_graph and self.hip_graphs and len(names) > 1):
            return False
        if train:
            self.model.train()
            self._ensure_flat_grad()
            if not self._fused:
                return False
        else:
            self.model.eval()
        self._ensure_arena()
        cs = tuple(self._resident(nm) for nm in names)
        if self._captured_lr != self._lr_signature():
            self._drop_graphs()
            self._captured_lr = self._lr_signature()
        kind = "epoch" if train else "epoch_eval"
        key = (tuple(names), kind)
        ent = self._graphs.get(key)
        if ent is None:
            ent = self._graphs[key] = self._capture(cs, kind)
        ent["graph"].replay()
        return True

    def _copy_groups(self, names):
        if not (self.epoch_graph and self.hip_graphs):
            return [[nm] for nm in names]
        left = sum(self._meta[nm][0] for nm in names)
        groups, cur, rows = [], [], 0
        for nm in names:
            cur.append(nm)
            rows += self._meta[nm][0]
            if 2 * rows >= left:
                groups.append(cur)
                left -= rows
                cur, rows = [], 0
        if cur:
            groups.append(cur)
        return groups

    def train_step(self, name: str):
        c = self._resident(name)
        self.model.train()
        self._ensure_flat_grad()
        self._ensure_arena()
        if self.multi:
            raise RuntimeError("use train_group() when running on more than one rank")
        if self._fused:
            return self._replay(c, "train") if self.hip_graphs else self._fwd_bwd_step(c)
        loss, probs, dx = self._replay(c, "fwdbwd") if self.hip_graphs else self._fwd_bwd(c)
        self._optimizer_step()
        return loss, probs, dx

    def eval_step(self, name: str):
        c = self._resident(name)
        self.model.eval()
        self._ensure_arena()
        if self.hip_graphs:
            loss, probs, _ = self._replay(c, "eval")
            return loss, probs
        return self._eval(c)

    def _warm_comms(self):
        if not self.multi or self._comm_warm:
            return
        torch.distributed.all_reduce(torch.zeros(1, device=self.device), group=self.group)
        if self.aux_group is not self.group:
            torch.distributed.all_reduce(torch.zeros(1, device=self.device), group=self.aux_group)
        self._comm_warm = True

    def train_group(self, name: Optional[str], group_size: int):
        self.model.train()
        self._ensure_flat_grad()
        self._ensure_arena()
        c = self._resident(name) if name is not None else None
        scale = 1.0 / group_size if group_size > 1 else 1.0
        self._warm_comms()
        if self._group_graph_enabled():
            try:
                return self._replay(c, "group", group_size)
            except Exception as e:
                import warnings
                warnings.warn("chromegcn_amd: capturing the step group (collective included) failed (%r); "
                              "using the captured fwd+bwd + stream-ordered collective + fused step instead" % (e,))
                self._group_graph_ok = False
                self._drop_graphs()
        out = (None, None, None)
        if c is not None:
            out = self._replay(c, "fwdbwd") if self.hip_graphs else self._fwd_bwd(c)
        else:
            self._flat_grad.zero_()
        if self.multi:
            self._allreduce_grads()
        self._optimizer_step(scale)
        return out

    def _group_graph_enabled(self) -> bool:
        if not (self.multi and self.hip_graphs and self._fused and self._group_graph_opt and self._group_graph_ok):
            return False
        return torch.distributed.get_backend(self.group) == "nccl"

    def _allreduce_grads(self):
        h = self._p2p
        if h is None:
            torch.distributed.all_reduce(self._flat_grad, op=torch.distributed.ReduceOp.SUM, group=self.group)
            return
        h.barrier(channel=0)
        acc = self._p2p_acc
        torch.add(self._p2p_views[0], self._p2p_views[1], out=acc) if len(self._p2p_views) > 1 else acc.copy_(self._p2p_views[0])
        for v in self._p2p_views[2:]:
            acc.add_(v)
        h.barrier(channel=1)
        self._flat_grad.copy_(acc)

    def _alloc_flat_grad(self, total, dev):
        self._p2p = None
        self.allreduce_kind = ({"nccl": "rccl"}.get(torch.distributed.get_backend(self.group), torch.distributed.get_backend(self.group))
                               if self.multi else "none")
        if self.multi and self._p2p_opt and dev.type == "cuda" and torch.distributed.get_backend(self.group) == "nccl":
            try:
                import torch.distributed._symmetric_memory as symm
                gname = (self.group or torch.distributed.group.WORLD).group_name
                buf = symm.empty(total, dtype=torch.float32, device=dev)
                buf.zero_()
                h = symm.rendezvous(buf, gname)
                self._p2p_views = [h.get_buffer(r, (total,), torch.float32) for r in range(h.world_size)]
                self._p2p_acc = torch.zeros(total, device=dev, dtype=torch.float32)
                self._p2p = h
                self.allreduce_kind = "p2p_one_shot"
                return buf
            except Exception as e:
                import warnings
                warnings.warn("chromegcn_amd: symmetric-memory P2P all-reduce unavailable (%r); using RCCL" % (e,))
        return torch.zeros(total, device=dev, dtype=torch.float32)

    def sync_running_stats(self, extra: Optional[torch.Tensor] = None, calls_total: int = 0, calls_mine: int = 0):
        if not self.multi:
            return extra
        bufs = [b for k, b in self.model.named_buffers() if b.dtype.is_floating_point]
        parts = [b.reshape(-1).float() for b in bufs]
        n_stat = sum(p.numel() for p in parts)
        if extra is not None:
            parts.append(extra.reshape(-1).float() * self.world)
        if not parts:
            return extra
        flat = torch.cat(parts)
        torch.distributed.all_reduce(flat, group=self.aux_group)
        flat.div_(self.world)
        off = 0
        for b in bufs:
            b.copy_(flat[off:off + b.numel()].view_as(b))
            off += b.numel()
        if calls_total:
            for k, b in self.model.named_buffers():
                if k.endswith("num_batches_tracked"):
                    b += int(calls_total - calls_mine)
        return flat[n_stat:].view_as(extra) if extra is not None else None

    def run_split(self, split: str, names: Optional[Sequence[str]] = None, to_cpu: bool = True, sync_loss: bool = True):
        names = list(self._meta) if names is None else list(names)
        train = split == "train"
        C = next(iter(self._meta.values()))[1] if self._meta else 0
        if not self.multi:
            self._ensure_arena()
            host = self._host_arena(C) if (to_cpu and names and self.device.type == "cuda") else None
            for grp in ([names] if host is None else self._copy_groups(names)):
                if not self._replay_epoch(grp, train):
                    for nm in grp:
                        self.train_step(nm) if train else self.eval_step(nm)
                if host is not None:
                    host.fetch([self._arena["rows"][nm] for nm in grp], self._arena["probs"])
            span = self._arena_span(names)
            if span is not None:
                preds_dev = self._arena["probs"][span[0]:span[1]]
                loss_dev = self._arena["loss"][span[2]:span[3]].sum()
            elif names:
                preds_dev = torch.cat([self._arena["slots"][nm]["probs"] for nm in names], 0)
                loss_dev = torch.cat([self._arena["slots"][nm]["loss"] for nm in names]).sum()
            else:
                preds_dev = torch.empty((0, C), device=self.device)
                loss_dev = torch.zeros((), device=self.device)
            total = float(loss_dev.item()) if (sync_loss or to_cpu) else loss_dev
            if not to_cpu:
                return preds_dev, self._split_targets_dev(names, C), total
            if host is not None:
                preds = host.finish(span, [self._arena["rows"][nm] for nm in names])
            else:
                preds = preds_dev.cpu()
        else:
            self._warm_comms()
            plan = plan_shards({nm: self._meta[nm][2] for nm in names}, self.world)
            ag = self.aux_group
            nccl = torch.distributed.get_backend(ag) == "nccl"
            mode = self.prediction_gather
            if mode == "rank0" and not nccl and self.device.type == "cuda":
                mode = "all"
            self.prediction_gather_effective = mode
            gp = self._gather_plan(names, plan, C, mode)
            peer = (lambda r: r) if ag is None else (lambda r: torch.distributed.get_global_rank(ag, r))
            loss_sum = torch.zeros((), device=self.device)
            pending = []
            for r, group in enumerate(plan.rounds):
                nm = group[self.rank] if self.rank < len(group) else None
                k = sum(1 for g in group if g is not None)
                if train:
                    loss, p, _ = self.train_group(nm, k)
                elif nm is not None:
                    loss, p = self.eval_step(nm)
                else:
                    loss = p = None
                if nm is not None:
                    loss_sum += loss
                if mode == "all":
                    send, recv = gp["send"][r], gp["recv"][r]
                    if nm is not None:
                        send[:p.shape[0]].copy_(p)
                    if nccl:
                        pending.append(torch.distributed.all_gather_into_tensor(recv, send, group=ag, async_op=True))
                    else:
                        pending.append(torch.distributed.all_gather(list(recv.view(self.world, -1, C).unbind(0)), send,
                                                                    group=ag, async_op=True))
                elif mode == "rank0":
                    ops = []
                    if self.rank == 0:
                        for src, g in enumerate(group):
                            if g is None:
                                continue
                            dst_rows = gp["rows"][g]
                            if src == 0:
                                dst_rows.copy_(p)
                            else:
                                ops.append(torch.distributed.P2POp(torch.distributed.irecv, dst_rows, peer(src), group=ag))
                    elif nm is not None:
                        ops.append(torch.distributed.P2POp(torch.distributed.isend, p, peer(0), group=ag))
                    if ops:
                        pending.extend(torch.distributed.batch_isend_irecv(ops))
            mine = sum(1 for nm in names if plan.owner[nm] == self.rank)
            S = 2
            if train:
                loss_sum = self.sync_running_stats(loss_sum, calls_total=S * len(names), calls_mine=S * mine)
            else:
                torch.distributed.all_reduce(loss_sum, group=ag)
            for w in pending:
                w.wait()
            total = float(loss_sum.item())
            if mode == "all":
                preds_dev = gp["recv_all"].index_select(0, gp["index"]) if gp["total"] else gp["recv_all"][:0]
            elif mode == "rank0":
# ... 100 lines not shown
```

chromegcn_amd/ops.py:

```python
from __future__ import annotations

import ctypes

import torch

from . import _lib
from . import graph as G
from .graph import ChromGraph

SUPPORTED_D = (128, 256)


def _require_cuda(t: torch.Tensor, name: str):
    if not t.is_cuda:
        raise RuntimeError(
            "chromegcn_amd: %s is on %s; the gated-GCN path only exists as HIP kernels "
            "(no CPU fallback) -- move the model and inputs to the GPU" % (name, t.device))
    if t.dtype != torch.float32:
        raise RuntimeError("chromegcn_amd: %s must be float32, got %s" % (name, t.dtype))


def _dense(t: torch.Tensor) -> torch.Tensor:
    t = t.contiguous()
    return t.clone() if t.data_ptr() % 16 else t


def _check_rng(rng_state, dropout: bool):
    if dropout and rng_state is None:
        raise RuntimeError("chromegcn_amd: fused dropout needs the model's rng_state tensor")


def _check_momentum(momentum):
    if momentum is None:
        raise RuntimeError("chromegcn_amd: BatchNorm momentum=None (cumulative average) is not supported by the fused head")


def _check_feat(x: torch.Tensor, g: ChromGraph, name="x", any_width=False):
    _require_cuda(x, name)
    ok_d = (x.dim() == 3 and x.shape[2] % 4 == 0 and 4 <= x.shape[2] <= 4096) if any_width else (x.dim() == 3 and x.shape[2] in SUPPORTED_D)
    if x.dim() != 3 or x.shape[0] not in (1, 2) or not ok_d:
        raise RuntimeError("chromegcn_amd: %s must be [S in {1,2}, n, d %s], got %s" %
                           (name, "a multiple of 4, <= 4096" if any_width else "in {128,256}", tuple(x.shape)))
    if x.shape[1] != g.n:
        raise RuntimeError("chromegcn_amd: %s has %d nodes but the graph has %d" % (name, x.shape[1], g.n))


def spmm(x, graph):
    _check_feat(x, graph, any_width=True)
    from . import torch_ops
    return torch.ops.chromegcn.spmm(x, graph.rowptr, graph.col, graph.val, graph.row_scale, graph.rowptr_t, graph.col_t,
                                    graph.val_t)


def sddmm(a, b, graph: ChromGraph, transposed=False, out=None):
    _check_feat(a, graph, "a")
    _check_feat(b, graph, "b")
    a, b = _dense(a), _dense(b)
    S, n, d = a.shape
    rowptr, col = (graph.rowptr_t, graph.col_t) if transposed else (graph.rowptr, graph.col)
    acc = out is not None
    if acc:
        if out.shape != (col.shape[0],) or out.dtype != torch.float32 or not out.is_contiguous() or out.device != a.device:
            raise RuntimeError("chromegcn_amd: sddmm accumulates into a contiguous fp32 [nnz] tensor on the features' device")
    else:
        out = torch.empty(col.shape[0], device=a.device, dtype=torch.float32)
    _lib.call("cgcn_sddmm", n=n, S=S, d=d, rowptr=rowptr, col=col, A=a, B=b, out=out, accumulate=1 if acc else 0)
    return out


def saliency_normalize(raw, graph: ChromGraph):
    _require_cuda(raw, "raw")
    raw = raw.contiguous()
    out = torch.empty_like(raw)
    _lib.call("cgcn_saliency_normalize", n=graph.n, rowptr=graph.rowptr, val=graph.val, raw=raw, out=out)
    return out


_EVAL_BWD_MSG = ("chromegcn_amd: backward through the fused classifier head needs train mode (the eval-mode kernel "
                 "saves nothing for it); call model.train(), or use ChromeGCN.forward / forward_strands, whose "
                 "torch head differentiates in eval mode like the reference's")

_saliency_tap = None

_sgd_fuse = None


def _sgd_fuse_arg(layer_id, sink):
    rq = _sgd_fuse
    if rq is None or rq.get("done") or layer_id != 1 or sink is None:
        return None
    fg = rq["grad"]
    lo, hi = fg.data_ptr(), fg.data_ptr() + 4 * fg.numel()
    if not all(lo <= t.data_ptr() and t.data_ptr() + 4 * t.numel() <= hi for t in sink):
        return None
    return _lib.SgdFuse(rq["param"].data_ptr(), fg.data_ptr(), _lib.ptr(rq["mom"]), fg.numel(), float(rq["lr"]),
                        float(rq["momentum"]), float(rq["weight_decay"]), float(rq["grad_scale"]), 1 if rq["nesterov"] else 0,
                        _lib.ptr(rq["rng_state"]))


def _layer_params(weight, bias, gate_w, gate_b):
    return _dense(weight), bias.contiguous(), gate_w.contiguous().view(-1), gate_b.contiguous().view(-1)


def _head_params(bn_w, bn_b, w_out, b_out):
    return _dense(bn_w), _dense(bn_b), _dense(w_out), b_out.contiguous()


def layer_fwd(x, params, csr, z, h, dropout_p=0.0, rng_state=None, layer_id=0, h_in=None, colstats=None, colstats_rows=0):
    S, n, d = x.shape
    weight, bias, wg, cg = params
    rowptr, col, val, row_scale = csr
    xn, gate = torch.empty_like(x), torch.empty((S, n), device=x.device, dtype=torch.float32)
    _lib.call("cgcn_layer_fwd", n=n, S=S, d=d, rowptr=rowptr, col=col, val=val, row_scale=row_scale, X=x, W=weight, b=bias,
              wg=wg, cg=cg, Xn=xn, Z=z, H=h, gate=gate, dropout_p=float(dropout_p),
              rng_state=rng_state if dropout_p > 0 else None, stream_id=int(layer_id), H_in=h_in, colstats=colstats,
              colstats_rows=colstats_rows, aux=G.aux_ptr(col))
    return xn, gate


def layer_bwd(x, z, h, gate, weight, wg, csr_t, dx, dhs, dropout_in, rng_state, layer_id, dxn=None, dgate=None, head=None,
              sink=None, fuse_sink=None, aux_stream=None):
    S, n, d = x.shape
    f32 = dict(device=x.device, dtype=torch.float32)
    if sink is not None:
        dw, db, dwg, dcg = sink
    else:
        dw, db, dwg, dcg = torch.empty_like(weight), torch.empty(d, **f32), torch.empty(d, **f32), torch.empty(1, **f32)
    ws = _lib.layer_bwd_workspace(n, S, d, x.device)
    sgd = _sgd_fuse_arg(layer_id, fuse_sink) if aux_stream is None else None
    rowptr_t, col_t, val_t, row_scale = csr_t
    _lib.call("cgcn_layer_bwd", n=n, S=S, d=d, rowptr_t=rowptr_t, col_t=col_t, val_t=val_t, row_scale=row_scale, X=x, Z=z,
              H=h, gate=gate, W=weight, wg=wg, dXn=dxn, dgate=dgate, dX=dx, dHs=dhs, dW=dw, db=db, dwg=dwg, dcg=dcg,
              accumulate=0, in_dropout_p=float(dropout_in), rng_state=rng_state, in_stream_id=max(layer_id - 1, 0),
              head=head, workspace=ws, workspace_bytes=ws.numel(), aux_stream=aux_stream, sgd=sgd, aux_t=G.aux_ptr(col_t))
    if sgd is not None:
        _sgd_fuse["done"] = True
    return dw, db, dwg, dcg


def head_fwd(x, params, target, run_mean, run_var, nbt, momentum, eps, training, dropout_p, rng_state, probs, loss, dpred,
             save_mean, save_invstd):
    S, n, d = x.shape
    bn_w, bn_b, w_out, b_out = params
    ws = _lib.head_workspace(n, S, d, w_out.shape[0], x.device)
    _lib.call("cgcn_head_fwd", n=n, S=S, d=d, C=w_out.shape[0], X=x, bn_w=bn_w, bn_b=bn_b, run_mean=run_mean, run_var=run_var,
              num_batches_tracked=nbt, momentum=float(momentum), eps=float(eps), training=1 if training else 0, W_out=w_out,
              b_out=b_out, target=target, dropout_p=float(dropout_p),
              rng_state=rng_state if training and dropout_p > 0 else None, probs=probs, loss=loss, dpred=dpred,
              save_mean=save_mean, save_invstd=save_invstd, workspace=ws, workspace_bytes=ws.numel())


def _head_grad_bufs(sink, d, w_out):
    if sink is not None:
        return sink
    f32 = dict(device=w_out.device, dtype=torch.float32)
    return torch.empty(d, **f32), torch.empty(d, **f32), torch.empty_like(w_out), torch.empty(w_out.shape[0], **f32)


def head_bwd(dloss, x, bn_w, bn_b, w_out, dpred, save_mean, save_invstd, dropout_p, rng_state, sink=None):
    S, n, d = x.shape
    C = w_out.shape[0]
    ws = _lib.head_workspace(n, S, d, C, x.device)
    dx = torch.empty_like(x)
    dbn_w, dbn_b, dw_out, db_out = _head_grad_bufs(sink, d, w_out)
    _lib.call("cgcn_head_bwd", n=n, S=S, d=d, C=C, X=x, bn_w=bn_w, bn_b=bn_b, save_mean=save_mean, save_invstd=save_invstd,
              W_out=w_out, dpred=dpred.contiguous(), dloss=dloss.contiguous().view(1), dropout_p=float(dropout_p),
              rng_state=rng_state if dropout_p > 0 else None, dX=dx, dW_out=dw_out, db_out=db_out, dbn_w=dbn_w, dbn_b=dbn_b,
              accumulate=0, workspace=ws, workspace_bytes=ws.numel())
    return dx, dbn_w, dbn_b, dw_out, db_out


_SPLIT_TABLE_BYTES = 6 << 20


def _resolve_h_cache(h_cache, x, need_bwd):
    if h_cache is not None and h_cache.get("h") is not None:
        hc = h_cache["h"]
        if hc.shape != x.shape or hc.device != x.device:
            raise RuntimeError("chromegcn_amd: cached aggregation does not match the input")
        return hc, None
    if need_bwd or h_cache is not None or (x.numel() * 4 >= _SPLIT_TABLE_BYTES and x.shape[0] * x.shape[2] <= 256):
        return None, torch.empty_like(x)
    return None, None


def _store_h_cache(h_cache, h_in, h):
    if h_in is not None:
        return h_in
    if h_cache is not None and h is not None:
        h_cache["h"] = h
    return h


def _out_slots(out_slots, n, C, device):
    if out_slots is not None:
        probs, loss = out_slots["probs"], out_slots["loss"]
        if tuple(probs.shape) != (n, C) or loss.numel() != 1 or not probs.is_contiguous() or probs.device != device:
            raise RuntimeError("chromegcn_amd: out_slots do not match [n, C] = [%d, %d]" % (n, C))
        return probs, loss.view(1)
    return (torch.empty((n, C), device=device, dtype=torch.float32), torch.empty(1, device=device, dtype=torch.float32))


def _sink_ok(sink, shapes):
    return sink is not None and all(t is not None and tuple(t.shape) == tuple(sh) and t.is_contiguous()
                                    for t, sh in zip(sink, shapes))


class GatedLayerFn(torch.autograd.Function):

    @staticmethod
    def forward(ctx, x, weight, bias, gate_w, gate_b, graph: ChromGraph, dropout_out, dropout_in, rng_state,
                layer_id, grad_sink, h_cache, zero_stat=None):
        _check_feat(x, graph)
        for t, nm in ((weight, "weight"), (bias, "bias"), (gate_w, "gate weight"), (gate_b, "gate bias")):
            _require_cuda(t, nm)
        x = _dense(x)
        S, n, d = x.shape
        if tuple(weight.shape) != (d, d):
            raise RuntimeError("chromegcn_amd: fused layer needs a square [d,d] weight, got %s" % (tuple(weight.shape),))
        params = _layer_params(weight, bias, gate_w, gate_b)
        need_bwd = any(ctx.needs_input_grad[:5])
        z = torch.empty_like(x) if need_bwd else None
        h_in, h = _resolve_h_cache(h_cache, x, need_bwd)
        _check_rng(rng_state, dropout_out > 0 or dropout_in > 0)
        xn, gate = layer_fwd(x, params, (graph.rowptr, graph.col, graph.val, graph.row_scale), z, h, dropout_out, rng_state,
                             layer_id, h_in, zero_stat, _lib.COLSTATS_ROWS_ZERO_ONLY if zero_stat is not None else 0)
        h = _store_h_cache(h_cache, h_in, h)
        if need_bwd:
            ctx.save_for_backward(x, z, h, gate, params[0], params[2], rng_state if dropout_in > 0 else None)
        ctx.graph = graph
        ctx.gate_w_shape = gate_w.shape
        ctx.gate_b_shape = gate_b.shape
        ctx.dropout_in = float(dropout_in)
        ctx.layer_id = int(layer_id)
        ctx.sink = grad_sink if _sink_ok(grad_sink, ((d, d), (d,), gate_w.shape, gate_b.shape)) else None
        ctx.set_materialize_grads(False)
        return xn, gate

    @staticmethod
    def backward(ctx, dxn, dgate):
        x, z, h, gate, weight, wg, rng_state = ctx.saved_tensors
        g = ctx.graph
        if dxn is None and dgate is None:
            return (None,) * 13
        dxn = torch.zeros_like(x) if dxn is None else _dense(dxn)
        dgate = None if dgate is None else dgate.contiguous()
        dx = torch.empty_like(x) if ctx.needs_input_grad[0] else None
        dhs = torch.empty_like(x) if (dx is not None or _saliency_tap is not None) else None
        dw, db, dwg, dcg = layer_bwd(x, z, h, gate, weight, wg, (g.rowptr_t, g.col_t, g.val_t, g.row_scale), dx, dhs,
                                     ctx.dropout_in, rng_state, ctx.layer_id, dxn, dgate, sink=ctx.sink, fuse_sink=ctx.sink,
                                     aux_stream=_lib.aux_stream_ptr())
        if _saliency_tap is not None:
            _saliency_tap.append((x, dhs, g))
        if ctx.sink is not None:
            return (dx, None, None, None, None) + (None,) * 8
        return (dx, dw, db, dwg.view(ctx.gate_w_shape), dcg.view(ctx.gate_b_shape)) + (None,) * 8


def gated_layer(x, weight, bias, gate_w, gate_b, graph, dropout_out=0.0, dropout_in=0.0, rng_state=None,
                layer_id=0, grad_sink=None, h_cache=None, zero_stat=None):
    if grad_sink is None and h_cache is None and _saliency_tap is None and zero_stat is None:
        _check_feat(x, graph)
        from . import torch_ops
        xn, gate, _z, _h = torch.ops.chromegcn.gated_layer(
            x, weight, bias, gate_w, gate_b, graph.rowptr, graph.col, graph.val, graph.row_scale, graph.rowptr_t,
            graph.col_t, graph.val_t, float(dropout_out), float(dropout_in), rng_state, int(layer_id))
        return xn, gate
    return GatedLayerFn.apply(x, weight, bias, gate_w, gate_b, graph, float(dropout_out), float(dropout_in),
                              rng_state, int(layer_id), grad_sink, h_cache, zero_stat)


def stat_buffer(x):
    S, n, d = x.shape
    rows = ctypes.c_int(0)
    tiles = _lib.query("cgcn_layer_fwd_colstats_plan", n=n, S=S, d=d, mode=_lib.COLSTATS_ACCUMULATE, rows_per_tile=rows)
    if tiles <= 0 or rows.value != -1:
        return None
    return torch.empty((tiles, S, d, 2), device=x.device, dtype=torch.float32)


class HeadLossFn(torch.autograd.Function):

    @staticmethod
    def forward(ctx, x, bn_w, bn_b, w_out, b_out, target, run_mean, run_var, nbt, momentum, eps, training,
                dropout_p, rng_state, grad_sink, out_slots=None):
        _require_cuda(x, "x")
        for t, nm in ((bn_w, "bn weight"), (bn_b, "bn bias"), (w_out, "out.weight"), (b_out, "out.bias"), (target, "target")):
            _require_cuda(t, nm)
        _check_momentum(momentum)
        x = _dense(x)
        S, n, d = x.shape
        C = w_out.shape[0]
        target = target.contiguous()
        if tuple(target.shape) != (n, C):
            raise RuntimeError("chromegcn_amd: target must be [n, C] = [%d, %d], got %s" % (n, C, tuple(target.shape)))
        params = _head_params(bn_w, bn_b, w_out, b_out)
        need_bwd = training and any(ctx.needs_input_grad[:5])
        ctx.eval_grad = (not training) and any(ctx.needs_input_grad[:5])
        probs, loss = _out_slots(out_slots, n, C, x.device)
        dpred = torch.empty((n, C), device=x.device, dtype=torch.float32) if need_bwd else None
        save_mean = torch.empty((S, d), device=x.device, dtype=torch.float32) if training else None
        save_invstd = torch.empty((S, d), device=x.device, dtype=torch.float32) if training else None
        drop = bool(training) and dropout_p > 0
        _check_rng(rng_state, drop)
        head_fwd(x, params, target, run_mean, run_var, nbt, momentum, eps, training, dropout_p, rng_state, probs, loss, dpred,
                 save_mean, save_invstd)
        if need_bwd:
            ctx.save_for_backward(x, *params[:3], dpred, save_mean, save_invstd, rng_state if drop else None)
            ctx.dropout_p = float(dropout_p) if drop else 0.0
            ctx.sink = grad_sink if _sink_ok(grad_sink, ((d,), (d,), (C, d), (C,))) else None
        ctx.mark_non_differentiable(probs)
        return loss.view(()), probs

    @staticmethod
    def backward(ctx, dloss, _dprobs):
        if ctx.eval_grad:
            raise RuntimeError(_EVAL_BWD_MSG)
        x, bn_w, bn_b, w_out, dpred, save_mean, save_invstd, rng_state = ctx.saved_tensors
        dx, dbn_w, dbn_b, dw_out, db_out = head_bwd(dloss, x, bn_w, bn_b, w_out, dpred, save_mean, save_invstd, ctx.dropout_p,
                                                    rng_state, ctx.sink)
        if ctx.sink is not None:
            return (dx,) + (None,) * 15
        return (dx, dbn_w, dbn_b, dw_out, db_out) + (None,) * 11


class LastLayerHeadLossFn(torch.autograd.Function):

    @staticmethod
    def forward(ctx, x, weight, bias, gate_w, gate_b, bn_w, bn_b, w_out, b_out, graph, target, run_mean, run_var, nbt,
                momentum, eps, training, dropout_p, dropout_in, rng_state, layer_id, layer_sink, head_sink, h_cache,
                out_slots=None, stat_acc=False, stat_buf=None):
        _check_feat(x, graph)
        for t, nm in ((weight, "weight"), (bias, "bias"), (gate_w, "gate weight"), (gate_b, "gate bias"),
                      (bn_w, "bn weight"), (bn_b, "bn bias"), (w_out, "out.weight"), (b_out, "out.bias"), (target, "target")):
            _require_cuda(t, nm)
        _check_momentum(momentum)
        x = _dense(x)
        S, n, d = x.shape
        C = w_out.shape[0]
        target = target.contiguous()
        if tuple(weight.shape) != (d, d) or tuple(target.shape) != (n, C):
            raise RuntimeError("chromegcn_amd: bad shapes for the fused last layer + head")
        weight, bias, wg, cg = _layer_params(weight, bias, gate_w, gate_b)
        bn_w, bn_b, w_out, b_out = _head_params(bn_w, bn_b, w_out, b_out)
        need_bwd = training and any(ctx.needs_input_grad[:9])
        ctx.eval_grad = (not training) and any(ctx.needs_input_grad[:9])
        z = torch.empty_like(x) if need_bwd else None
        h_in, h = _resolve_h_cache(h_cache, x, need_bwd)
        colstats, cs_tiles, cs_rows, fwd_rows = None, 0, 0, 0
        if need_bwd:
            if stat_acc and stat_buf is not None:
                colstats, cs_tiles, cs_rows = stat_buf, stat_buf.shape[0], -1
                fwd_rows = _lib.COLSTATS_ROWS_ACCUMULATE_ZEROED
            else:
                mode = _lib.COLSTATS_ACCUMULATE if (stat_acc and (h is not None or h_in is not None)) else _lib.COLSTATS_RECORDS
                rows = ctypes.c_int(0)
                cs_tiles = _lib.query("cgcn_layer_fwd_colstats_plan", n=n, S=S, d=d, mode=mode, rows_per_tile=rows)
                cs_rows = fwd_rows = rows.value
                colstats = torch.empty((cs_tiles, S, d, 2), device=x.device, dtype=torch.float32)
        xn, gate = layer_fwd(x, (weight, bias, wg, cg), (graph.rowptr, graph.col, graph.val, graph.row_scale), z, h,
                             layer_id=layer_id, h_in=h_in, colstats=colstats, colstats_rows=fwd_rows)
        h = _store_h_cache(h_cache, h_in, h)
        probs, loss = _out_slots(out_slots, n, C, x.device)
        save_mean = torch.empty((S, d), device=x.device, dtype=torch.float32) if training else None
        save_invstd = torch.empty((S, d), device=x.device, dtype=torch.float32) if training else None
        drop = bool(training) and dropout_p > 0
        _check_rng(rng_state, drop or dropout_in > 0)
        if need_bwd:
            ws = _lib.head_workspace(n, S, d, C, x.device)
            _lib.call("cgcn_head_train", n=n, S=S, d=d, C=C, X=xn, bn_w=bn_w, bn_b=bn_b, run_mean=run_mean, run_var=run_var,
                      num_batches_tracked=nbt, momentum=float(momentum), eps=float(eps), W_out=w_out, b_out=b_out,
                      target=target, dropout_p=float(dropout_p) if drop else 0.0, rng_state=rng_state if drop else None,
                      probs=probs, loss=loss, save_mean=save_mean, save_invstd=save_invstd, col_stats=colstats,
                      col_stats_tiles=cs_tiles, col_stats_rows=cs_rows, workspace=ws, workspace_bytes=ws.numel())
        else:
            head_fwd(xn, (bn_w, bn_b, w_out, b_out), target, run_mean, run_var, nbt, momentum, eps, training, dropout_p,
                     rng_state, probs, loss, None, save_mean, save_invstd)
        if need_bwd:
            ctx.save_for_backward(x, z, h, gate, weight, wg, xn, bn_w, bn_b, w_out, ws, save_mean, save_invstd,
                                  rng_state if (drop or dropout_in > 0) else None,
                                  colstats if cs_rows == -1 else None)
            ctx.graph = graph
            ctx.dropout_p = float(dropout_p) if drop else 0.0
            ctx.dropout_in = float(dropout_in)
            ctx.layer_id = int(layer_id)
            ctx.shapes = (gate_w.shape, gate_b.shape)
            ctx.layer_sink = layer_sink if _sink_ok(layer_sink, ((d, d), (d,), gate_w.shape, gate_b.shape)) else None
            ctx.head_sink = head_sink if _sink_ok(head_sink, ((d,), (d,), (C, d), (C,))) else None
        ctx.mark_non_differentiable(probs, gate)
        ctx.set_materialize_grads(False)
        return loss.view(()), probs, gate

    @staticmethod
    def backward(ctx, dloss, _dprobs, _dgate):
        if ctx.eval_grad:
            raise RuntimeError(_EVAL_BWD_MSG)
        if dloss is None:
            return (None,) * 27
        (x, z, h, gate, weight, wg, xn, bn_w, bn_b, w_out, hws, save_mean, save_invstd, rng_state, stat_acc) = ctx.saved_tensors
        g = ctx.graph
        S, n, d = x.shape
        C = w_out.shape[0]
        dbn_w, dbn_b, dw_out, db_out = _head_grad_bufs(ctx.head_sink, d, w_out)
        dloss = dloss.contiguous().view(1)
        o_dym, o_bnc, o_part = ctypes.c_size_t(), ctypes.c_size_t(), ctypes.c_size_t()
        _lib.call("cgcn_head_workspace_layout", n=n, S=S, d=d, C=C, dym_offset=o_dym, bnc_offset=o_bnc, part_offset=o_part)
        hg = _lib.HeadGrad(hws.data_ptr() + o_dym.value, hws.data_ptr() + o_bnc.value, save_mean.data_ptr(),
                           save_invstd.data_ptr(), bn_w.data_ptr(), ctx.dropout_p, _lib.ptr(rng_state),
                           hws.data_ptr() + o_part.value, _lib.query("cgcn_head_bwd_partials", n=n), C, dw_out.data_ptr(),
                           db_out.data_ptr(), 0, dloss.data_ptr(), dbn_w.data_ptr(), dbn_b.data_ptr(), _lib.ptr(stat_acc))
        dx = torch.empty_like(x) if ctx.needs_input_grad[0] else None
        dhs = torch.empty_like(x) if dx is not None else None
        dw, db, dwg, dcg = layer_bwd(x, z, h, gate, weight, wg, (g.rowptr_t, g.col_t, g.val_t, g.row_scale), dx, dhs,
                                     ctx.dropout_in, rng_state, ctx.layer_id, head=hg, sink=ctx.layer_sink,
                                     fuse_sink=ctx.layer_sink if ctx.head_sink is not None else None,
                                     aux_stream=_lib.aux_stream_ptr())
        gl = (None,) * 4 if ctx.layer_sink is not None else (dw, db, dwg.view(ctx.shapes[0]), dcg.view(ctx.shapes[1]))
        gh = (None,) * 4 if ctx.head_sink is not None else (dbn_w, dbn_b, dw_out, db_out)
        return (dx,) + gl + gh + (None,) * 18


def last_layer_head_loss(x, gc, wk, bn, out, graph, target, training, dropout_p, dropout_in, rng_state, layer_id,
                         layer_sink=None, head_sink=None, h_cache=None, out_slots=None, stat_acc=False, stat_buf=None):
    return LastLayerHeadLossFn.apply(x, gc.weight, gc.bias, wk.weight, wk.bias, bn.weight, bn.bias, out.weight, out.bias,
                                     graph, target, bn.running_mean, bn.running_var, bn.num_batches_tracked, bn.momentum,
                                     bn.eps, bool(training), float(dropout_p), float(dropout_in), rng_state, int(layer_id),
                                     layer_sink, head_sink, h_cache, out_slots, bool(stat_acc), stat_buf)


def head_loss(x, bn: torch.nn.BatchNorm1d, out: torch.nn.Linear, target, training, dropout_p, rng_state, grad_sink=None,
              out_slots=None):
    if grad_sink is None and out_slots is None:
        from . import torch_ops
        _require_cuda(x, "x")
        return torch_ops.head_loss_module(x, bn, out, target, training, dropout_p, rng_state)
    return HeadLossFn.apply(x, bn.weight, bn.bias, out.weight, out.bias, target, bn.running_mean, bn.running_var,
                            bn.num_batches_tracked, bn.momentum, bn.eps, bool(training), float(dropout_p), rng_state,
# ... 75 lines not shown
```

include/chromegcn.h:

```cpp
#ifndef CHROMEGCN_H
#define CHROMEGCN_H

#include <stddef.h>
#include <stdint.h>

#ifdef __cplusplus
extern "C" {
#endif

#define CGCN_OK 0
#define CGCN_ERR_BAD_ARG (-1)
#define CGCN_ERR_UNSUPPORTED (-2)
#define CGCN_ERR_LAUNCH (-3)
#define CGCN_ERR_WORKSPACE (-4)

#define CGCN_ABI_VERSION 26

typedef void *cgcn_stream_t;

typedef struct cgcn_graph_aux {
  const uint16_t *col16;
  const int32_t *row_order;
  int32_t max_row_len;
  int32_t band_halfwidth;
  const int32_t *bp_rowptr;
  const int32_t *bp_col;
  const uint16_t *bp_col16;
  const int32_t *bp_row_order;
} cgcn_graph_aux;

int cgcn_abi_version(void);

const char *cgcn_strerror(int code);

int cgcn_spmm(cgcn_stream_t stream, int n_rows, int n_cols, int S, int d,
              const int32_t *rowptr, const int32_t *col, const float *val, const float *row_scale,
              const float *X, float *Y, const cgcn_graph_aux *aux);

int cgcn_layer_fwd(cgcn_stream_t stream, int n, int S, int d,
                   const int32_t *rowptr, const int32_t *col, const float *val, const float *row_scale,
                   const float *X, const float *W, const float *b, const float *wg, const float *cg,
                   float *Xn, float *Z, float *H, float *gate,
                   float dropout_p, const unsigned long long *rng_state, unsigned int stream_id,
                   const float *H_in, float *colstats, int colstats_rows, const cgcn_graph_aux *aux);

#define CGCN_COLSTATS_RECORDS 0
#define CGCN_COLSTATS_ACCUMULATE 1
#define CGCN_COLSTATS_ROWS_ACCUMULATE (-1)
#define CGCN_COLSTATS_ROWS_ZERO_ONLY (-2)
#define CGCN_COLSTATS_ROWS_ACCUMULATE_ZEROED (-3)

int cgcn_layer_fwd_colstats_plan(int n, int S, int d, int mode, int *rows_per_tile);

void cgcn_debug_set_fwd_split_bytes(long long bytes);

#define CGCN_PRODUCTS_FP32_CHAIN 0
#define CGCN_PRODUCTS_SPLIT 1
void cgcn_debug_set_products(int mode);
int cgcn_debug_get_products(void);

int cgcn_debug_layer_fwd_route(int n, int S, int d, const cgcn_graph_aux *aux, int colstats_rows);
int cgcn_debug_layer_bwd_route(int n, int S, int d);

typedef struct cgcn_head_grad {
  const float *dym;
  const float *bnc;
  const float *save_mean;
  const float *save_invstd;
  const float *bn_w;
  float dropout_p;
  const unsigned long long *rng_state;
  const float *part;
  int n_partials;
  int C;
  float *dW_out;
  float *db_out;
  int accumulate;
  const float *dloss;
  float *dbn_w;
  float *dbn_b;
  const void *stat_acc;
} cgcn_head_grad;

typedef struct cgcn_sgd_fuse {
  float *param;
  const float *grad;
  float *momentum_buf;
  long long count;
  float lr, momentum, weight_decay, grad_scale;
  int nesterov;
  unsigned long long *rng_state;
} cgcn_sgd_fuse;

size_t cgcn_layer_bwd_workspace_bytes(int n, int S, int d);

int cgcn_layer_bwd(cgcn_stream_t stream, int n, int S, int d,
                   const int32_t *rowptr_t, const int32_t *col_t, const float *val_t, const float *row_scale,
                   const float *X, const float *Z, const float *H, const float *gate,
                   const float *W, const float *wg,
                   const float *dXn, const float *dgate,
                   float *dX, float *dHs, float *dW, float *db, float *dwg, float *dcg,
                   int accumulate, float in_dropout_p, const unsigned long long *rng_state,
                   unsigned int in_stream_id, const cgcn_head_grad *head,
                   void *workspace, size_t workspace_bytes, cgcn_stream_t aux_stream,
                   const cgcn_sgd_fuse *sgd, const cgcn_graph_aux *aux_t);

int cgcn_debug_layer_bwd_phases(cgcn_stream_t stream, int n, int S, int d,
                                const int32_t *rowptr_t, const int32_t *col_t, const float *val_t, const float *row_scale,
                                const float *X, const float *Z, const float *H, const float *gate,
                                const float *W, const float *wg, const float *dXn, const float *dgate,
                                float *dX, float *dHs, float *dW, float *db, float *dwg, float *dcg,
                                int accumulate, float in_dropout_p, const unsigned long long *rng_state,
                                unsigned int in_stream_id, const cgcn_head_grad *head,
                                void *workspace, size_t workspace_bytes, int phases, const cgcn_graph_aux *aux_t);

size_t cgcn_head_workspace_bytes(int n, int S, int d, int C);

int cgcn_head_workspace_layout(int n, int S, int d, int C, size_t *dym_offset, size_t *bnc_offset,
                               size_t *part_offset);
int cgcn_head_bwd_partials(int n);

int cgcn_head_fwd(cgcn_stream_t stream, int n, int S, int d, int C, const float *X, const float *bn_w,
                  const float *bn_b, float *run_mean, float *run_var, long long *num_batches_tracked,
                  float momentum, float eps, int training, const float *W_out, const float *b_out,
                  const float *target, float dropout_p, const unsigned long long *rng_state,
                  float *probs, float *loss, float *dpred, float *save_mean, float *save_invstd,
                  void *workspace, size_t workspace_bytes);

int cgcn_head_logits(cgcn_stream_t stream, int n, int S, int d, int C, const float *X, const float *bn_w,
                     const float *bn_b, const float *run_mean, const float *run_var, float eps, const float *W_out,
                     const float *b_out, float *logits);

int cgcn_head_train(cgcn_stream_t stream, int n, int S, int d, int C, const float *X, const float *bn_w,
                    const float *bn_b, float *run_mean, float *run_var, long long *num_batches_tracked,
                    float momentum, float eps, const float *W_out, const float *b_out, const float *target,
                    float dropout_p, const unsigned long long *rng_state, float *probs, float *loss,
                    float *save_mean, float *save_invstd, const float *col_stats, int col_stats_tiles,
                    int col_stats_rows, void *workspace, size_t workspace_bytes);

int cgcn_debug_head_train_phases(cgcn_stream_t stream, int n, int S, int d, int C, const float *X, const float *bn_w,
                                 const float *bn_b, float *run_mean, float *run_var, long long *num_batches_tracked,
                                 float momentum, float eps, const float *W_out, const float *b_out, const float *target,
                                 float dropout_p, const unsigned long long *rng_state, float *probs, float *loss,
                                 float *save_mean, float *save_invstd, const float *col_stats, int col_stats_tiles,
                                 int col_stats_rows, void *workspace, size_t workspace_bytes, int phases);

int cgcn_head_bwd(cgcn_stream_t stream, int n, int S, int d, int C, const float *X, const float *bn_w,
                  const float *bn_b, const float *save_mean, const float *save_invstd, const float *W_out,
                  const float *dpred, const float *dloss, float dropout_p, const unsigned long long *rng_state,
                  float *dX, float *dW_out, float *db_out, float *dbn_w, float *dbn_b, int accumulate,
                  void *workspace, size_t workspace_bytes);

int cgcn_sddmm(cgcn_stream_t stream, int n, int S, int d, const int32_t *rowptr, const int32_t *col,
               const float *A, const float *B, float *out, int accumulate);

int cgcn_saliency_normalize(cgcn_stream_t stream, int n, const int32_t *rowptr, const float *val, const float *raw, float *out);

#define CGCN_ADJ_HIC 0
#define CGCN_ADJ_CONSTANT 1
#define CGCN_ADJ_BOTH 2
#define CGCN_ADJ_NONE 3

int cgcn_graph_count(cgcn_stream_t stream, int n, int adj_type, const int32_t *rowptr_in, const int32_t *col_in,
                     const float *val_in, int32_t *row_counts, int32_t *rowptr_out);

int cgcn_graph_fill(cgcn_stream_t stream, int n, int adj_type, const int32_t *rowptr_in, const int32_t *col_in,
                    const float *val_in, const int32_t *rowptr_out, int32_t *col_out, float *val_out,
                    float *row_scale, int32_t *symmetric_flag);

size_t cgcn_metrics_workspace_bytes(long long n, int C);

int cgcn_multilabel_metrics(cgcn_stream_t stream, long long n, int C, const float *probs, const float *targets,
                            float fdr_cutoff, float *out, void *workspace, size_t workspace_bytes);

int cgcn_multilabel_metrics_nonneg(cgcn_stream_t stream, long long n, int C, const float *probs, const float *targets,
                                   float fdr_cutoff, float *out, int32_t *bad, void *workspace, size_t workspace_bytes);

int cgcn_sgd_step(cgcn_stream_t stream, long long count, float *param, const float *grad, float *momentum_buf,
                  float lr, float momentum, float weight_decay, int nesterov, float grad_scale,
                  unsigned long long *rng_state);

int cgcn_adam_step(cgcn_stream_t stream, long long count, float *param, const float *grad, float *exp_avg,
                   float *exp_avg_sq, float *step, int n_step, int32_t *ticket, float lr, float beta1, float beta2,
                   float eps, float weight_decay, float grad_scale, unsigned long long *rng_state);

int cgcn_ablation_prepare(cgcn_stream_t stream, int n, int C, const float *targets, uint32_t *label_bits,
                          int32_t *pos_lists, int32_t *pos_ranks, int32_t *pos_counts);

size_t cgcn_ablation_workspace_bytes(int n_inst, int S, int d, int layers);

int cgcn_ablation_layer(cgcn_stream_t stream, int n, int S, int d, const int32_t *rowptr, const int32_t *col,
                        const float *val, const float *row_scale, const float *X, const float *X_inst, const float *W,
                        const float *b, const float *wg, const float *cg, const uint32_t *label_bits, int C,
                        const int32_t *pos_list, const int32_t *pos_rank, int n_pos, const int32_t *cols, int n_cols,
                        float *X_out, int32_t *removed);

int cgcn_ablation_head(cgcn_stream_t stream, int n, int S, int d, int C, const float *X, const float *X_inst,
                       const float *bn_w, const float *bn_b, const float *run_mean, const float *run_var, float eps,
                       const float *W_out, const float *b_out, const int32_t *pos_lists, const int32_t *pos_counts,
                       int label, int n_pos, const int32_t *cols, int n_cols, const int32_t *removed, float *base,
                       float *M);

int cgcn_ablation_mask(cgcn_stream_t stream, int n, int C, const int32_t *rowptr, const int32_t *col, const float *val,
                       const float *row_scale, const uint32_t *label_bits, int label_i, int label_j, float *val_out,
                       float *row_scale_out, int32_t *removed);

int cgcn_ablation_reduce(cgcn_stream_t stream, int n, int S, int C, const float *logits, const int32_t *pos_lists,
                         const int32_t *pos_counts, int label, int col_label, const int32_t *removed, float *base,
                         float *M);

size_t cgcn_hic_workspace_bytes(long long M, int N, long long capacity, long long K);

int cgcn_hic_count(cgcn_stream_t stream, long long M, const int32_t *pos1, const int32_t *pos2,
                   const int32_t *window_start, int N, void *workspace, size_t workspace_bytes, long long *n_survivors);

int cgcn_hic_build(cgcn_stream_t stream, long long M, const int32_t *pos1, const int32_t *pos2, const double *count,
                   const double *norm, long long n_bins, int resolution_bp, const int32_t *window_start, int N,
                   long long K, long long capacity, void *workspace, size_t workspace_bytes, int32_t *rowptr_out,
                   int32_t *col_out, int32_t *nnz_out, long long *n_survivors);

size_t cgcn_hic_up_workspace_bytes(long long M, int N, long long capacity, long long K, int resolution_bp, int window_bp,
                                   long long n_window_bins);

int cgcn_hic_count_up(cgcn_stream_t stream, long long M, const int32_t *pos1, const int32_t *pos2,
                      const int32_t *window_start, int N, int resolution_bp, int window_bp, long long n_window_bins,
                      void *workspace, size_t workspace_bytes, long long *n_survivors);

int cgcn_hic_build_up(cgcn_stream_t stream, long long M, const int32_t *pos1, const int32_t *pos2, const double *count,
                      const double *norm, long long n_bins, int resolution_bp, int window_bp, long long n_window_bins,
                      const int32_t *window_start, int N, long long K, long long capacity, void *workspace,
                      size_t workspace_bytes, int32_t *rowptr_out, int32_t *col_out, int32_t *nnz_out,
                      long long *n_survivors);

#define CGCN_TEXT_LINE_MAX 64
#define CGCN_TEXT_SLOW 1
#define CGCN_TEXT_MALFORMED 2

size_t cgcn_text_workspace_bytes(long long n_bytes);

int cgcn_text_count(cgcn_stream_t stream, const void *text, long long n_bytes, void *workspace, size_t workspace_bytes,
                    long long *n_records);

int cgcn_text_parse(cgcn_stream_t stream, const void *text, long long n_bytes, long long M, int32_t *pos1_out,
                    int32_t *pos2_out, double *count_out, long long *flags, long long flag_capacity,
                    long long *flag_totals, void *workspace, size_t workspace_bytes);

#ifdef __cplusplus
}
#endif
#endif
```

Before: 59.33 million.

## Fuse next chromosome's input aggregation into layer-1 backward kernel grid

Adds a companion SpMM job that lets the first-layer input aggregation of the next chromosome run as extra blocks inside the current chromosome's layer-1 backward sliced kernel. The aggregated result is handed off to the next step's forward in place of recomputing it. The aim is to fill idle GPU capacity in the tail of the backward gather kernel and save a separate launch. The cost is extra buffers per chromosome, more complex grid partitioning with rider blocks, and possible interference with the backward blocks' memory bandwidth.

Result: faster. 60.65 million (median of 6 runs) (+2.2%).

```diff
diff --git a/chromegcn_amd/_lib.py b/chromegcn_amd/_lib.py
--- a/chromegcn_amd/_lib.py
+++ b/chromegcn_amd/_lib.py
@@ -31,6 +31,10 @@
     "cgcn_debug_layer_bwd_phases": (_c_int, "stream n:i S:i d:i rowptr_t col_t val_t row_scale X Z H gate W wg dXn dgate dX dHs "
                                             "dW db dwg dcg accumulate:i in_dropout_p:f rng_state in_stream_id:u head workspace "
                                             "workspace_bytes:z phases:i aux_t"),
+    "cgcn_layer_bwd_co": (_c_int, "stream n:i S:i d:i rowptr_t col_t val_t row_scale X Z H gate W wg dXn dgate dX dHs dW db "
+                                  "dwg dcg accumulate:i in_dropout_p:f rng_state in_stream_id:u head workspace "
+                                  "workspace_bytes:z aux_stream sgd aux_t companion"),
+    "cgcn_debug_layer_bwd_co_route": (_c_int, "n:i S:i d:i rowptr_t col_t val_t have_dX:i aux_t companion"),
     "cgcn_head_workspace_bytes": (_c_sz, "n:i S:i d:i C:i"),
     "cgcn_head_workspace_layout": (_c_int, "n:i S:i d:i C:i dym_offset:zp bnc_offset:zp part_offset:zp"),
     "cgcn_head_bwd_partials": (_c_int, "n:i"),
@@ -194,6 +198,11 @@
                 ("nesterov", _c_int), ("rng_state", _c_vp)]
 
 
+class SpmmJob(ctypes.Structure):
+    _fields_ = [("n", _c_int), ("S", _c_int), ("d", _c_int), ("rowptr", _c_vp), ("col", _c_vp), ("val", _c_vp),
+                ("row_scale", _c_vp), ("X", _c_vp), ("H", _c_vp), ("aux", _c_vp)]
+
+
 def ptr(t):
     return None if t is None else t.data_ptr()
 
diff --git a/chromegcn_amd/csrc/cgcn_kernels.hip b/chromegcn_amd/csrc/cgcn_kernels.hip
--- a/chromegcn_amd/csrc/cgcn_kernels.hip
+++ b/chromegcn_amd/csrc/cgcn_kernels.hip
@@ -2117,24 +2117,18 @@
   return a;
 }
 
-template <int S, int D, bool HAS_VAL, typename IT = int, bool BP = false>
-__global__ __launch_bounds__(512) __attribute__((amdgpu_waves_per_eu(HAS_VAL ? 6 : 8))) void k_aggregate_sliced(int n, const int* __restrict__ rowptr, const IT* __restrict__ col,
-                                                          const float* __restrict__ val, const float* __restrict__ rs,
-                                                          const float* __restrict__ X, float* __restrict__ H,
-                                                          const int* __restrict__ order,
-                                                          unsigned long long* __restrict__ zero_words, int zero_count) {
-  static_assert(!(BP && HAS_VAL), "the band-plus CSR holds unit entries");
+template <int S, int D, bool HAS_VAL, typename IT, bool BP>
+__device__ __forceinline__ void aggregate_sliced_tile(int b, int n, const int* __restrict__ rowptr, const IT* __restrict__ col,
+                                                      const float* __restrict__ val, const float* __restrict__ rs,
+                                                      const float* __restrict__ X, float* __restrict__ H,
+                                                      const int* __restrict__ order, f32x4* __restrict__ bt) {
   constexpr int NSL = S * D / 32, QPR = D / 32;
   const int lane = threadIdx.x & 63, wave = threadIdx.x >> 6;
-  const int zblocks = (int)gridDim.x < 8 ? (int)gridDim.x : 8;
-  if (zero_words && (int)blockIdx.x < zblocks)
-    for (int i = (int)blockIdx.x * 512 + (int)threadIdx.x; i < zero_count; i += zblocks * 512) zero_words[i] = 0ull;
   int slice, tile;
-  sliced_block<NSL>(blockIdx.x, (n + 63) / 64, slice, tile);
+  sliced_block<NSL>(b, (n + 63) / 64, slice, tile);
   const size_t slice_el = (size_t)(slice / QPR) * n * D + (slice % QPR) * 32;
   const size_t lane_el = slice_el + (lane & 7) * 4;
   const SlicedTile t = sliced_tile(rowptr, order, n, tile, wave, lane);
-  __shared__ f32x4 bt[BP ? BANDPLUS_CHUNKS : 1];
   if (BP) {
     bandplus_stage(bt, X, slice_el, n, t.g0, D);
     __syncthreads();
@@ -2151,6 +2145,20 @@
   }
 }
 
+template <int S, int D, bool HAS_VAL, typename IT = int, bool BP = false>
+__global__ __launch_bounds__(512) __attribute__((amdgpu_waves_per_eu(HAS_VAL ? 6 : 8))) void k_aggregate_sliced(int n, const int* __restrict__ rowptr, const IT* __restrict__ col,
+                                                          const float* __restrict__ val, const float* __restrict__ rs,
+                                                          const float* __restrict__ X, float* __restrict__ H,
+                                                          const int* __restrict__ order,
+                                                          unsigned long long* __restrict__ zero_words, int zero_count) {
+  static_assert(!(BP && HAS_VAL), "the band-plus CSR holds unit entries");
+  const int zblocks = (int)gridDim.x < 8 ? (int)gridDim.x : 8;
+  if (zero_words && (int)blockIdx.x < zblocks)
+    for (int i = (int)blockIdx.x * 512 + (int)threadIdx.x; i < zero_count; i += zblocks * 512) zero_words[i] = 0ull;
+  __shared__ f32x4 bt[BP ? BANDPLUS_CHUNKS : 1];
+  aggregate_sliced_tile<S, D, HAS_VAL, IT, BP>(blockIdx.x, n, rowptr, col, val, rs, X, H, order, bt);
+}
+
 template <int S, int D, bool EXT = false>
 __device__ __forceinline__ void bwd_riders(int extra, int n, int P, const float* __restrict__ part, float* __restrict__ dW,
                                            float* __restrict__ db, float* __restrict__ dwg, float* __restrict__ dcg,
@@ -2173,6 +2181,20 @@
   }
   sgd_other_elements(sg, extra - head_slabs, D, dW, db, dwg, dcg);
 }
+
+#ifndef CO_AGG_LAST
+#define CO_AGG_LAST 0
+#endif
+struct CoAgg {
+  int n, start, blocks, riders, riders_end;
+  const int* rowptr;
+  const void* col;
+  const float* val;
+  const float* rs;
+  const float* X;
+  float* H;
+  const int* order;
+};
 
 template <int S, int D, bool HAS_VAL, typename IT = int, bool BP = false>
 __global__ __launch_bounds__(512) __attribute__((amdgpu_waves_per_eu(HAS_VAL ? 6 : 8))) void k_bwd_sliced(int n, const int* __restrict__ rowptr, const IT* __restrict__ col,
@@ -2184,12 +2206,18 @@
                                                     const float* __restrict__ part, float* __restrict__ dW,
                                                     float* __restrict__ db, float* __restrict__ dwg,
                                                     float* __restrict__ dcg, int accumulate, SgdFuse sg, int reduce_slabs,
-                                                    const int* __restrict__ order, HeadApply hp, int head_slabs) {
+                                                    const int* __restrict__ order, HeadApply hp, int head_slabs, CoAgg co) {
   constexpr int RIDER_STAGE = 4 * (512 / HEAD_STAT_COLS) * (HEAD_STAT_COLS + 1) * (int)sizeof(double) / 16;
   __shared__ f32x4 bt[BP ? (BANDPLUS_CHUNKS > RIDER_STAGE ? BANDPLUS_CHUNKS : RIDER_STAGE) : 1];
   if ((int)blockIdx.x >= gather_blocks) {
+    const int b = (int)blockIdx.x;
+    if ((unsigned)(b - co.start) < (unsigned)co.blocks) {
+      aggregate_sliced_tile<S, D, HAS_VAL, IT, BP>(b - co.start, co.n, co.rowptr, (const IT*)co.col, co.val, co.rs, co.X, co.H, co.order, bt);
+      return;
+    }
 #ifndef BSX_NORIDERS
-    bwd_riders<S, D, BP>((int)blockIdx.x - gather_blocks, n, P, part, dW, db, dwg, dcg, accumulate, sg, reduce_slabs, hp, head_slabs, bt);
+    if (b >= co.riders && b < co.riders_end)
+      bwd_riders<S, D, BP>(b - co.riders, n, P, part, dW, db, dwg, dcg, accumulate, sg, reduce_slabs, hp, head_slabs, bt);
 #endif
     return;
   }
@@ -2650,8 +2678,7 @@
   else hipLaunchKernelGGL((k_band_aggregate<2, 256, BAND_R>), dim3(blocks), dim3(512), 0, st, n, rs, X, H, zw, zc);
 }
 
-int cgcn_spmm(cgcn_stream_t stream, int n_rows, int n_cols, int S, int d, const int32_t* rowptr, const int32_t* col,
-              const float* val, const float* row_scale, const float* X, float* Y, const cgcn_graph_aux* aux) {
+static int spmm_check(int n_rows, int n_cols, int S, int d, const int32_t* rowptr, const int32_t* col, const float* X, const float* Y) {
   const int nmax = n_rows > n_cols ? n_rows : n_cols;
   if (nmax < 0) return CGCN_ERR_BAD_ARG;
   if (!(S == 1 || S == 2) || d < 4 || (d & 3) || d > 4096) return CGCN_ERR_UNSUPPORTED;
@@ -2659,6 +2686,17 @@
   if (n_rows == 0) return CGCN_OK;
   if (!rowptr || !col || !X || !Y || X == Y) return CGCN_ERR_BAD_ARG;
   if (misaligned16(X) || misaligned16(Y)) return CGCN_ERR_BAD_ARG;
+  return CGCN_OK;
+}
+static inline bool spmm_sliced_route(int n, int S, int d, const float* val, const cgcn_graph_aux* aux) {
+  return (d == 128 || d == 256) && !band_graph(aux, val) &&
+         ((double)n * S * d * 4.0 >= (double)g_fwd_split_bytes.load() || hub_graph(aux) || bandplus_graph(aux, val));
+}
+
+int cgcn_spmm(cgcn_stream_t stream, int n_rows, int n_cols, int S, int d, const int32_t* rowptr, const int32_t* col,
+              const float* val, const float* row_scale, const float* X, float* Y, const cgcn_graph_aux* aux) {
+  const int crc = spmm_check(n_rows, n_cols, S, d, rowptr, col, X, Y);
+  if (crc || n_rows == 0) return crc;
   hipStream_t st = (hipStream_t)stream;
   if (!(d == 128 || d == 256)) {
     const long long rows = (long long)S * n_rows;
@@ -2670,7 +2708,7 @@
     launch_band_aggregate(st, n_rows, S, d, row_scale, X, Y);
     return launch_status();
   }
-  if (n_rows == n_cols && ((double)n_rows * S * d * 4.0 >= (double)g_fwd_split_bytes.load() || hub_graph(aux) || bandplus_graph(aux, val))) {
+  if (n_rows == n_cols && spmm_sliced_route(n_rows, S, d, val, aux)) {
     const int gblocks = (S * d / 32) * ((n_rows + 63) / 64);
     const SlicedCsr c = sliced_csr(aux, rowptr, col, val, n_cols);
     launch_aggregate_sliced(st, gblocks, n_rows, S, d, c.rowptr, c.col, c.col16, c.val, row_scale, X, Y, c.order, c.bp);
@@ -2850,16 +2888,31 @@
   return (size_t)bwd_partials(n, S, d) * ((size_t)d * d + 2 * d + 4) * sizeof(float);
 }
 
+static bool companion_rides(const cgcn_spmm_job* co, int S, int d, const SlicedCsr& main) {
+  if (co->S != S || co->d != d || S * d / 32 > 8 || !spmm_sliced_route(co->n, S, d, co->val, co->aux)) return false;
+  const SlicedCsr cc = sliced_csr(co->aux, co->rowptr, co->col, co->val, co->n);
+  return cc.bp == main.bp && (cc.col16 != nullptr) == (main.col16 != nullptr) && (cc.val != nullptr) == (main.val != nullptr);
+}
+
 static int layer_bwd_impl(cgcn_stream_t stream, int n, int S, int d, const int32_t* rowptr_t, const int32_t* col_t,
                           const float* val_t, const float* row_scale, const float* X, const float* Z, const float* H,
                           const float* gate, const float* W, const float* wg, const float* dXn, const float* dgate, float* dX,
                           float* dHs, float* dW, float* db, float* dwg, float* dcg, int accumulate, float in_dropout_p,
                           const unsigned long long* rng_state, unsigned int in_stream_id, const cgcn_head_grad* head,
                           void* workspace, size_t workspace_bytes, cgcn_stream_t aux_stream, const cgcn_sgd_fuse* sgd,
-                          int phases, const cgcn_graph_aux* aux_t) {
+                          int phases, const cgcn_graph_aux* aux_t, const cgcn_spmm_job* co = nullptr) {
   int rc = check_shape(n, S, d);
   if (rc) return rc;
   if (!rowptr_t || !col_t || !X || !Z || !H || !gate || !W || !wg || !dW || !db || !dwg || !dcg) return CGCN_ERR_BAD_ARG;
+  if (co) {
+    if ((rc = spmm_check(co->n, co->n, co->S, co->d, co->rowptr, co->col, co->X, co->H))) return rc;
+    if (co->n == 0) co = nullptr;
+  }
+  if (co) {
+    const void* mine[] = {X, Z, H, gate, W, wg, dXn, dgate, dX, dHs, dW, db, dwg, dcg, workspace, row_scale};
+    for (const void* q : mine)
+      if (q && q == (const void*)co->H) return CGCN_ERR_BAD_ARG;
+  }
   if (dX && !dHs) return CGCN_ERR_BAD_ARG;
   SgdFuse sg = {nullptr, nullptr, nullptr, 0, 0.f, 0.f, 0.f, 1.f, 0, nullptr};
   if (sgd) {
@@ -2941,9 +2994,12 @@
     if ((rc = launch_status())) return rc;
     if (rs_stream != st && hipEventRecord(ev_join, rs_stream) != hipSuccess) return CGCN_ERR_LAUNCH;
   }
+  auto companion_alone = [&]() -> int {
+    return co ? cgcn_spmm(stream, co->n, co->n, co->S, co->d, co->rowptr, co->col, co->val, co->row_scale, co->X, co->H, co->aux) : CGCN_OK;
+  };
   if (n == 0 || !dX) {
     if (rs_stream != st && hipStreamWaitEvent(st, ev_join, 0) != hipSuccess) return CGCN_ERR_LAUNCH;
-    return CGCN_OK;
+    return companion_alone();
   }
   const int blocks = (S * d / 32) * ((n + 63) / 64);
   if (head) dXn = dX;
@@ -2959,40 +3015,53 @@
     else if (S == 1 && d == 256) CALLB(1, 256);
     else CALLB(2, 256);
 #undef CALLB
-  } else if (bandplus_graph(aux_t, val_t)) {
+  } else {
     const SlicedCsr c = sliced_csr(aux_t, rowptr_t, col_t, val_t, n);
-#define CALLBP(S_, D_, IT_, COL_)                                                                                    \
-  hipLaunchKernelGGL((k_bwd_sliced<S_, D_, false, IT_, true>), dim3(blocks + (fuse_reduce ? rslabs : 0) + head_slabs_g + sgd_blocks), dim3(512), 0, \
-                     st, n, c.rowptr, COL_, nullptr, dHs, dXn, gate, dX, ks, th, rng_state, in_stream_id, blocks, P,  \
-                     part, dW, db, dwg, dcg, accumulate, sg, fuse_reduce ? rslabs : 0, c.order, hp, head_slabs_g)
-#define CALLBP16(S_, D_) CALLBP(S_, D_, uint16_t, c.col16)
-#define CALLBP32(S_, D_) CALLBP(S_, D_, int, c.col)
-    if (c.col16) { if (S == 1 && d == 128) CALLBP16(1, 128); else if (S == 2 && d == 128) CALLBP16(2, 128); else if (S == 1 && d == 256) CALLBP16(1, 256); else CALLBP16(2, 256); }
-    else { if (S == 1 && d == 128) CALLBP32(1, 128); else if (S == 2 && d == 128) CALLBP32(2, 128); else if (S == 1 && d == 256) CALLBP32(1, 256); else CALLBP32(2, 256); }
+    const int nriders = (fuse_reduce ? rslabs : 0) + head_slabs_g + sgd_blocks;
+    CoAgg ca = {0, 0, 0, blocks, blocks + nriders, nullptr, nullptr, nullptr, nullptr, nullptr, nullptr, nullptr};
+    int grid = blocks + nriders;
+    if (co && rs_stream == st && companion_rides(co, S, d, c)) {
+      const SlicedCsr cc = sliced_csr(co->aux, co->rowptr, co->col, co->val, co->n);
+      const int cblocks = (S * d / 32) * ((co->n + 63) / 64);
+#if CO_AGG_LAST
+      ca.start = (blocks + nriders + 7) & ~7;
+#else
+      ca.start = (blocks + 7) & ~7;
+      ca.riders = ca.start + cblocks;
+      ca.riders_end = ca.riders + nriders;
+#endif
+      ca.n = co->n;
+      ca.blocks = cblocks;
+      ca.rowptr = cc.rowptr;
+      ca.col = cc.col16 ? (const void*)cc.col16 : (const void*)cc.col;
+      ca.val = cc.val;
+      ca.rs = co->row_scale;
+      ca.X = co->X;
+      ca.H = co->H;
+      ca.order = cc.order;
+      grid = (ca.start + cblocks > ca.riders_end) ? ca.start + cblocks : ca.riders_end;
+      co = nullptr;
+    }
+#define BSL(S_, D_, V_, IT_, BP_, COL_)                                                                               \
+  hipLaunchKernelGGL((k_bwd_sliced<S_, D_, V_, IT_, BP_>), dim3(grid), dim3(512), 0, st, n, c.rowptr, COL_, c.val, dHs, dXn, gate, dX, \
+                     ks, th, rng_state, in_stream_id, blocks, P, part, dW, db, dwg, dcg, accumulate, sg, fuse_reduce ? rslabs : 0, \
+                     c.order, hp, head_slabs_g, ca)
+#define CALLBP16(S_, D_) BSL(S_, D_, false, uint16_t, true, c.col16)
+#define CALLBP32(S_, D_) BSL(S_, D_, false, int, true, c.col)
+#define CALL16(S_, D_) BSL(S_, D_, false, uint16_t, false, c.col16)
+#define CALL(S_, D_, V_) BSL(S_, D_, V_, int, false, c.col)
+    if (c.bp) { if (c.col16) SD4(CALLBP16); else SD4(CALLBP32); }
+    else if (c.col16) SD4(CALL16);
+    else DISPATCH_SDV(S, d, c.val != nullptr, CALL);
+#undef CALL
+#undef CALL16
+#undef CALLBP32
 #undef CALLBP16
-#undef CALLBP32
-#undef CALLBP
-  } else if (const uint16_t* col16_t = use_col16(aux_t, val_t, n)) {
-#define CALL16(S_, D_)                                                                                               \
-  hipLaunchKernelGGL((k_bwd_sliced<S_, D_, false, uint16_t>), dim3(blocks + (fuse_reduce ? rslabs : 0) + head_slabs_g + sgd_blocks), dim3(512), 0, \
-                     st, n, rowptr_t, col16_t, val_t, dHs, dXn, gate, dX, ks, th, rng_state, in_stream_id, blocks, P, \
-                     part, dW, db, dwg, dcg, accumulate, sg, fuse_reduce ? rslabs : 0, row_order(aux_t), hp, head_slabs_g)
-    if (S == 1 && d == 128) CALL16(1, 128);
-    else if (S == 2 && d == 128) CALL16(2, 128);
-    else if (S == 1 && d == 256) CALL16(1, 256);
-    else CALL16(2, 256);
-#undef CALL16
-  } else {
-#define CALL(S_, D_, V_)                                                                                             \
-  hipLaunchKernelGGL((k_bwd_sliced<S_, D_, V_, int>), dim3(blocks + (fuse_reduce ? rslabs : 0) + head_slabs_g + sgd_blocks), dim3(512), 0, \
-                     st, n, rowptr_t, col_t, val_t, dHs, dXn, gate, dX, ks, th, rng_state, in_stream_id, blocks, P,  \
-                     part, dW, db, dwg, dcg, accumulate, sg, fuse_reduce ? rslabs : 0, row_order(aux_t), hp, head_slabs_g)
-    DISPATCH_SDV(S, d, val_t != nullptr, CALL);
-#undef CALL
+#undef BSL
   }
   if ((rc = launch_status())) return rc;
   if (rs_stream != st && hipStreamWaitEvent(st, ev_join, 0) != hipSuccess) return CGCN_ERR_LAUNCH;
-  return CGCN_OK;
+  return companion_alone();
 }
 
 int cgcn_layer_bwd(cgcn_stream_t stream, int n, int S, int d, const int32_t* rowptr_t, const int32_t* col_t,
@@ -3005,6 +3074,28 @@
   return layer_bwd_impl(stream, n, S, d, rowptr_t, col_t, val_t, row_scale, X, Z, H, gate, W, wg, dXn, dgate, dX, dHs, dW, db,
                         dwg, dcg, accumulate, in_dropout_p, rng_state, in_stream_id, head, workspace, workspace_bytes,
                         aux_stream, sgd, 3, aux_t);
+}
+
+int cgcn_layer_bwd_co(cgcn_stream_t stream, int n, int S, int d, const int32_t* rowptr_t, const int32_t* col_t,
+                      const float* val_t, const float* row_scale, const float* X, const float* Z, const float* H,
+                      const float* gate, const float* W, const float* wg, const float* dXn, const float* dgate, float* dX,
+                      float* dHs, float* dW, float* db, float* dwg, float* dcg, int accumulate, float in_dropout_p,
+                      const unsigned long long* rng_state, unsigned int in_stream_id, const cgcn_head_grad* head,
+                      void* workspace, size_t workspace_bytes, cgcn_stream_t aux_stream, const cgcn_sgd_fuse* sgd,
+                      const cgcn_graph_aux* aux_t, const cgcn_spmm_job* companion) {
+  return layer_bwd_impl(stream, n, S, d, rowptr_t, col_t, val_t, row_scale, X, Z, H, gate, W, wg, dXn, dgate, dX, dHs, dW, db,
+                        dwg, dcg, accumulate, in_dropout_p, rng_state, in_stream_id, head, workspace, workspace_bytes,
+                        aux_stream, sgd, 3, aux_t, companion);
+}
+
+int cgcn_debug_layer_bwd_co_route(int n, int S, int d, const int32_t* rowptr_t, const int32_t* col_t, const float* val_t,
+                                  int have_dX, const cgcn_graph_aux* aux_t, const cgcn_spmm_job* companion) {
+  int rc = check_shape(n, S, d);
+  if (rc) return rc;
+  if (!companion) return 0;
+  if ((rc = spmm_check(companion->n, companion->n, companion->S, companion->d, companion->rowptr, companion->col, companion->X, companion->H))) return rc;
+  if (n == 0 || companion->n == 0 || !have_dX || band_graph(aux_t, val_t)) return 0;
+  return companion_rides(companion, S, d, sliced_csr(aux_t, rowptr_t, col_t, val_t, n)) ? 1 : 0;
 }
 
 int cgcn_debug_layer_bwd_phases(cgcn_stream_t stream, int n, int S, int d, const int32_t* rowptr_t, const int32_t* col_t,
diff --git a/chromegcn_amd/finetune.py b/chromegcn_amd/finetune.py
--- a/chromegcn_amd/finetune.py
+++ b/chromegcn_amd/finetune.py
@@ -115,6 +115,9 @@
         self.model = model
         self.stat_acc = stat_acc if stat_acc is not None else (None if os.environ.get("CGCN_STAT_ACC", "1") != "0" else False)
         self.epoch_graph = epoch_graph if epoch_graph is not None else os.environ.get("CGCN_EPOCH_GRAPH", "1") != "0"
+        self.co_aggregation = os.environ.get("CGCN_CO_AGG", "1") != "0"
+        self._h1_co: Dict[str, torch.Tensor] = {}
+        self._h1_handoff: Dict[str, dict] = {}
         if prediction_gather not in ("all", "rank0", "none"):
             raise ValueError("prediction_gather must be 'all', 'rank0' or 'none'")
         self.prediction_gather = prediction_gather
@@ -169,6 +172,7 @@
     def _drop_graphs(self):
         self._graphs.clear()
         self._pool = None
+        self._h1_co.clear()
 
     def add_chromosome(self, name: str, feats: Dict[str, torch.Tensor], hic=None, defer: bool = False):
         n = feats["forward"].shape[0]
@@ -441,7 +445,7 @@
         slot = self._arena["slots"][c.name] if self._arena is not None else None
         if self.fused_head and hasattr(self.model, "forward_loss"):
             loss, probs, _ = self.model.forward_loss(x, c.graph, c.target,
-                                                     h1_cache=c.h1 if self.cache_input_aggregation else None,
+                                                     h1_cache=self._h1_handoff.get(c.name, c.h1 if self.cache_input_aggregation else None),
                                                      out_slots=slot, stat_acc=c.stat_acc)
             return loss, probs
         logits, _ = self.model.forward_strands(x, c.graph)
@@ -454,8 +458,35 @@
             slot["loss"].copy_(loss.detach().view(1))
         return loss, slot["probs"]
 
-    def _fwd_bwd_step(self, c: _Chrom):
+    def _co_agg_plan(self, cs):
+        plan = [False] * len(cs)
+        if not (self.co_aggregation and self.input_grad and not self.cache_input_aggregation and self.fused_head
+                and hasattr(self.model, "forward_loss") and getattr(self.model, "n_layers", 0) >= 2):
+            return plan
+        for k in range(1, len(cs)):
+            cc = cs[k]
+            S, n, d = cc.x.shape
+            plan[k] = _lib_mod.query("cgcn_debug_layer_fwd_route", n=n, S=S, d=d, aux=G.aux_ptr(cc.graph.col), colstats_rows=0) == 1
+            buf = self._h1_co.get(cc.name)
+            if plan[k] and (buf is None or buf.shape != cc.x.shape or buf.device != cc.x.device):
+                self._h1_co[cc.name] = torch.empty_like(cc.x)
+        return plan
+
+    def _fwd_bwd_step(self, c: _Chrom, co_next: Optional[_Chrom] = None):
         from . import ops
+        if co_next is not None:
+            buf = self._h1_co[co_next.name]
+            ops._co_agg = {"job": ops.spmm_job(co_next.x, co_next.graph, buf), "done": False}
+            try:
+                out = self._fwd_bwd_step(c)
+                if not ops._co_agg["done"]:
+                    g = co_next.graph
+                    _lib_mod.call("cgcn_spmm", n_rows=g.n, n_cols=g.n, S=buf.shape[0], d=buf.shape[2], rowptr=g.rowptr, col=g.col,
+                              val=g.val, row_scale=g.row_scale, X=co_next.x, Y=buf, aux=G.aux_ptr(g.col))
+            finally:
+                ops._co_agg = None
+            self._h1_handoff[co_next.name] = {"h": buf}
+            return out
         fuse = self._fused == "sgd" and getattr(self.model, "_grad_sink", False) and getattr(self.model, "n_layers", 0) >= 1
         if fuse:
             g = self.optimizer.param_groups[0]
@@ -523,12 +554,17 @@
         was_training = self.model.training
         self.model.train(kind not in ("eval", "epoch_eval"))
         snap = self._snapshot()
+        co_plan = self._co_agg_plan(c) if kind == "epoch" else None
 
         def body(collective=True):
             if kind in ("epoch", "epoch_eval"):
                 out = None
-                for cc in c:
-                    out = self._fwd_bwd_step(cc) if kind == "epoch" else self._eval(cc) + (None,)
+                try:
+                    for k, cc in enumerate(c):
+                        nxt = c[k + 1] if (co_plan is not None and k + 1 < len(c) and co_plan[k + 1]) else None
+                        out = self._fwd_bwd_step(cc, nxt) if kind == "epoch" else self._eval(cc) + (None,)
+                finally:
+                    self._h1_handoff.clear()
                 return out
             if kind == "eval":
                 loss, probs = self._eval(c)
diff --git a/chromegcn_amd/ops.py b/chromegcn_amd/ops.py
--- a/chromegcn_amd/ops.py
+++ b/chromegcn_amd/ops.py
@@ -98,6 +98,15 @@
                         _lib.ptr(rq["rng_state"]))
 
 
+_co_agg = None
+
+
+def spmm_job(x, graph, h):
+    S, n, d = x.shape
+    return _lib.SpmmJob(n, S, d, _lib.ptr(graph.rowptr), _lib.ptr(graph.col), _lib.ptr(graph.val), _lib.ptr(graph.row_scale),
+                        x.data_ptr(), h.data_ptr(), G.aux_ptr(graph.col))
+
+
 def _layer_params(weight, bias, gate_w, gate_b):
     return _dense(weight), bias.contiguous(), gate_w.contiguous().view(-1), gate_b.contiguous().view(-1)
 
@@ -129,10 +138,16 @@
     ws = _lib.layer_bwd_workspace(n, S, d, x.device)
     sgd = _sgd_fuse_arg(layer_id, fuse_sink) if aux_stream is None else None
     rowptr_t, col_t, val_t, row_scale = csr_t
-    _lib.call("cgcn_layer_bwd", n=n, S=S, d=d, rowptr_t=rowptr_t, col_t=col_t, val_t=val_t, row_scale=row_scale, X=x, Z=z,
-              H=h, gate=gate, W=weight, wg=wg, dXn=dxn, dgate=dgate, dX=dx, dHs=dhs, dW=dw, db=db, dwg=dwg, dcg=dcg,
-              accumulate=0, in_dropout_p=float(dropout_in), rng_state=rng_state, in_stream_id=max(layer_id - 1, 0),
-              head=head, workspace=ws, workspace_bytes=ws.numel(), aux_stream=aux_stream, sgd=sgd, aux_t=G.aux_ptr(col_t))
+    co = _co_agg if (layer_id == 1 and _co_agg is not None and not _co_agg["done"]) else None
+    args = dict(n=n, S=S, d=d, rowptr_t=rowptr_t, col_t=col_t, val_t=val_t, row_scale=row_scale, X=x, Z=z,
+                H=h, gate=gate, W=weight, wg=wg, dXn=dxn, dgate=dgate, dX=dx, dHs=dhs, dW=dw, db=db, dwg=dwg, dcg=dcg,
+                accumulate=0, in_dropout_p=float(dropout_in), rng_state=rng_state, in_stream_id=max(layer_id - 1, 0),
+                head=head, workspace=ws, workspace_bytes=ws.numel(), aux_stream=aux_stream, sgd=sgd, aux_t=G.aux_ptr(col_t))
+    if co is None:
+        _lib.call("cgcn_layer_bwd", **args)
+    else:
+        _lib.call("cgcn_layer_bwd_co", companion=co["job"], **args)
+        co["done"] = True
     if sgd is not None:
         _sgd_fuse["done"] = True
     return dw, db, dwg, dcg
diff --git a/include/chromegcn.h b/include/chromegcn.h
--- a/include/chromegcn.h
+++ b/include/chromegcn.h
@@ -114,6 +114,31 @@
                                 unsigned int in_stream_id, const cgcn_head_grad *head,
                                 void *workspace, size_t workspace_bytes, int phases, const cgcn_graph_aux *aux_t);
 
+typedef struct cgcn_spmm_job {
+  int n, S, d;
+  const int32_t *rowptr;
+  const int32_t *col;
+  const float *val;
+  const float *row_scale;
+  const float *X;
+  float *H;
+  const cgcn_graph_aux *aux;
+} cgcn_spmm_job;
+
+int cgcn_layer_bwd_co(cgcn_stream_t stream, int n, int S, int d,
+                      const int32_t *rowptr_t, const int32_t *col_t, const float *val_t, const float *row_scale,
+                      const float *X, const float *Z, const float *H, const float *gate,
+                      const float *W, const float *wg,
+                      const float *dXn, const float *dgate,
+                      float *dX, float *dHs, float *dW, float *db, float *dwg, float *dcg,
+                      int accumulate, float in_dropout_p, const unsigned long long *rng_state,
+                      unsigned int in_stream_id, const cgcn_head_grad *head,
+                      void *workspace, size_t workspace_bytes, cgcn_stream_t aux_stream,
+                      const cgcn_sgd_fuse *sgd, const cgcn_graph_aux *aux_t, const cgcn_spmm_job *companion);
+
+int cgcn_debug_layer_bwd_co_route(int n, int S, int d, const int32_t *rowptr_t, const int32_t *col_t, const float *val_t,
+                                  int have_dX, const cgcn_graph_aux *aux_t, const cgcn_spmm_job *companion);
+
 size_t cgcn_head_workspace_bytes(int n, int S, int d, int C);
 
 int cgcn_head_workspace_layout(int n, int S, int d, int C, size_t *dym_offset, size_t *bnc_offset,
```
